# fgnt/padertorch

Measured on AMD Instinct MI355X. Metric: training frames/sec (PIT mask-est, 2-spk 8 kHz), higher is better.
Workload: dtype f32

## Files before the change

include/ptmi.h:

```cpp
#ifndef PTMI_H_
#define PTMI_H_

#include <stdint.h>

#ifdef __cplusplus
extern "C" {
#endif

#define PTMI_OK 0
#define PTMI_E_INVALID (-1)
#define PTMI_E_UNSUPPORTED (-2)

typedef void* ptmi_stream_t;

const char* ptmi_version(void);
const char* ptmi_error_string(int code);

typedef struct ptmi_stft_geom {
    int32_t size;
    int32_t shift;
    int32_t window_length;
    int32_t pad_left;
    int32_t pad_right;
    int32_t pad;
// ... 111 lines not shown
int ptmi_unit_norm_backward(const float* gy, const float* y, const float* inv_norm, float* dx, int64_t N, int32_t E,
                            int32_t F, float eps, ptmi_stream_t stream);

int64_t ptmi_td_stats_elems(int32_t K);
int64_t ptmi_td_workspace_elems(int64_t batch, int32_t K, int64_t T);
int ptmi_td_pair_stats(const float* est, const float* tgt, const int32_t* lengths, int64_t batch, int32_t K,
                       int64_t T, const int64_t* strides, double* workspace, double* stats,
                       ptmi_stream_t stream);
int ptmi_td_lincomb(const float* x, const float* y, const int32_t* lengths, const float* coef_a,
                    const float* coef_b, const float* coef_c, int64_t batch, int32_t K, int64_t T,
                    const int64_t* strides, float* out, ptmi_stream_t stream);

int ptmi_tas_analysis(const float* x, const float* weight, const float* bias, float* out, int64_t B, int64_t T, int32_t N,
                      int32_t L, int32_t stride, int64_t E, int32_t relu, ptmi_stream_t stream);
int ptmi_tas_synthesis(const float* p, const float* mask, const float* gate, const float* weight, const float* bias, float* y,
                       int32_t K, int64_t B, int32_t N, int32_t L, int32_t stride, int64_t E, int64_t T_out,
                       ptmi_stream_t stream);
int ptmi_tas_masked_decode_backward(const float* gy, const float* mask, const float* encoded, const float* weight, float* dmask,
                                    float* dencoded, int32_t K, int64_t B, int64_t T, int32_t N, int32_t L, int32_t stride,
                                    int64_t E, ptmi_stream_t stream);
int64_t ptmi_tas_wgrad_workspace_elems(int64_t B, int32_t N, int32_t L, int32_t stride, int64_t E);
int ptmi_tas_wgrad(const float* g, const float* mask, const float* gate, const float* x, int32_t K, int64_t B, int64_t T,
                   int32_t N, int32_t L, int32_t stride, int64_t E, float* workspace, float* out, ptmi_stream_t stream);

int64_t ptmi_tcn_depthwise_workspace_elems(int64_t B, int64_t T, int32_t H, int32_t K);
int ptmi_tcn_depthwise_forward(const float* u, const float* slope_in, const float* weight, const float* bias, const float* slope_out,
                               float* v, float* stats, double* workspace, int64_t B, int64_t T, int32_t H, int32_t K,
                               int32_t dilation, float eps, ptmi_stream_t stream);
int ptmi_tcn_depthwise_backward(const float* gv, const float* u, const float* slope_in, const float* weight, const float* bias,
                                const float* slope_out, float* gz, float* gu, float* dparams, double* workspace, int64_t B,
                                int64_t T, int32_t H, int32_t K, int32_t dilation, ptmi_stream_t stream);
int64_t ptmi_tcn_norm_workspace_elems(int64_t B, int64_t T, int32_t C);
int ptmi_tcn_norm_stats(const float* x, float* stats, double* workspace, int64_t B, int64_t T, int32_t C, int32_t rows, float eps,
                        ptmi_stream_t stream);
int ptmi_tcn_norm_apply(const float* x, const float* stats, const float* gamma, const float* beta, float* y, int64_t B, int64_t T,
                        int32_t C, int32_t rows, ptmi_stream_t stream);
int ptmi_tcn_norm_backward(const float* gy, const float* x, const float* stats, const float* gamma, float* dx, float* dparams,
                           float* gsum, double* workspace, int64_t B, int64_t T, int32_t C, int32_t rows, ptmi_stream_t stream);

int64_t ptmi_tasnet_entry_norm_workspace_elems(int64_t B, int32_t N, int64_t E);
int ptmi_tasnet_entry_norm_forward(const float* w, const float* gamma, const float* beta, const void* lengths, int32_t lengths_int64,
                                   float* y, float* stats, int64_t B, int32_t N, int64_t E, float eps, ptmi_stream_t stream);
int ptmi_tasnet_entry_norm_backward(const float* gy, const float* w, const float* stats, const float* gamma, const void* lengths,
                                    int32_t lengths_int64, float* dw, float* dparams, double* workspace, int64_t B, int32_t N,
                                    int64_t E, ptmi_stream_t stream);
int64_t ptmi_tasnet_prelu_workspace_elems(int64_t n);
int ptmi_tasnet_prelu_forward(const float* x, const float* slope, float* y, int64_t n, ptmi_stream_t stream);
int ptmi_tasnet_prelu_backward(const float* g, const float* x, const float* slope, float* gx, float* dslope, double* workspace,
                               int64_t n, ptmi_stream_t stream);
int ptmi_tasnet_mask_head_forward(const float* z, float* m, float* additional, int64_t B, int64_t E, int32_t N, int32_t K, int32_t A,
                                  int32_t activation, ptmi_stream_t stream);
int ptmi_tasnet_mask_head_backward(const float* gm, const float* m, const float* g_additional, float* gz, int64_t B, int64_t E,
                                   int32_t N, int32_t K, int32_t A, int32_t activation, ptmi_stream_t stream);
int64_t ptmi_tasnet_center_workspace_elems(int64_t K, int64_t B, int64_t T_in, int64_t T_out);
int ptmi_tasnet_center(const float* in, float* out, double* workspace, int64_t K, int64_t B, int64_t T_in, int64_t T_out,
                       int32_t backward, ptmi_stream_t stream);

int64_t ptmi_dprnn_num_chunks(int64_t L, int32_t K, int32_t P);
int ptmi_dprnn_tables(const void* lengths, int32_t lengths_int64, int32_t B, int32_t S, int32_t K, int32_t P, int32_t* chunks,
                      int32_t* intra, int32_t* inter, ptmi_stream_t stream);
int32_t ptmi_chunk_lstm_max_hidden(void);
int32_t ptmi_chunk_lstm_max_resident_hidden(void);
int32_t ptmi_chunk_lstm_tile(void);
int ptmi_chunk_lstm_forward(float* gates, const float* w_hh, const float* w_hh_reverse, const float* b_hh, const float* b_hh_reverse,
                            float* h, float* c, const int32_t* table, int32_t nseq, int32_t cap, int32_t H, int32_t ndir,
                            ptmi_stream_t stream);
int ptmi_chunk_lstm_backward(float* gates, const float* dh, const float* w_hh, const float* w_hh_reverse, const float* h, const float* c,
                             float* hprev, const int32_t* table, int32_t nseq, int32_t cap, int32_t H, int32_t ndir,
                             ptmi_stream_t stream);
int64_t ptmi_dprnn_colsum_workspace_elems(int64_t rows, int32_t C);
int ptmi_dprnn_colsum(const float* x, int64_t ld, float* out, float* out2, double* workspace, int64_t rows, int32_t C,
                      ptmi_stream_t stream);
int ptmi_dprnn_norm_residual_forward(const float* z, const float* residual, const float* gamma, const float* beta,
                                     const int32_t* chunks, float* y, float* stats, int64_t rows, int32_t N, int32_t S, int32_t K,
                                     float eps, ptmi_stream_t stream);
int ptmi_dprnn_norm_residual_backward(const float* gy, const float* z, const float* stats, const float* gamma, const int32_t* chunks,
                                      float* dz, float* dresidual, float* dparams, double* workspace, int64_t rows, int32_t N,
                                      int32_t S, int32_t K, ptmi_stream_t stream);
int ptmi_dprnn_segment(const float* x, const int64_t* x_strides, float* seg, int64_t B, int64_t L, int32_t N, int32_t S, int32_t K,
                       int32_t P, ptmi_stream_t stream);
int ptmi_dprnn_overlap_add(const float* seg, const int64_t* seg_strides, float* out, int64_t B, int64_t L_out, int32_t N, int32_t S,
                           int32_t K, int32_t P, int32_t front, ptmi_stream_t stream);

int64_t ptmi_td_rect_workspace_elems(int64_t batch, int32_t M, int32_t K, int64_t T);
int ptmi_td_rect_stats(const float* est, const float* tgt, int64_t batch, int32_t M, int32_t K, int64_t T, const int64_t* strides,
                       double* workspace, double* stats, double* gram, ptmi_stream_t stream);
int ptmi_orpit_select(const double* stats, const double* gram, const int32_t* alive_in, int32_t* alive_out, float* loss,
                      int32_t* choice, float* coef_a, float* coef_b, int64_t batch, int32_t K, int64_t n, ptmi_stream_t stream);
int ptmi_td_rect_lincomb(const float* est, const float* tgt, const float* g, const float* coef_a, const float* coef_b, int64_t batch,
                         int32_t M, int32_t K, int64_t T, const int64_t* strides, float* out, ptmi_stream_t stream);
int64_t ptmi_orpit_flag_workspace_elems(int64_t B, int32_t A, int64_t E);
int ptmi_orpit_flag_forward(const float* additional, const float* weight, const float* bias, const float* mask, const float* encoded,
                            float* pre, float* w, float* flag, double* stat, double* workspace, int64_t B, int32_t A, int64_t E,
                            int32_t N, int32_t K, int32_t k, int32_t weighted, ptmi_stream_t stream);
int ptmi_orpit_flag_backward(const float* gflag, const float* gpre, const float* flag, const double* stat, const float* pre, const float* w,
                             const float* additional, const float* weight, const float* mask, const float* encoded, float* dadditional,
                             float* dparams, float* dmask, float* dencoded, double* workspace, int64_t B, int32_t A, int64_t E, int32_t N,
                             int32_t K, int32_t k, int32_t weighted, ptmi_stream_t stream);

int64_t ptmi_bf_psd_workspace_elems(int64_t B, int32_t C, int64_t T, int64_t F, int32_t M);
int ptmi_bf_psd(const float* Y, const float* mask0, const float* mask1, const int32_t* frames, int64_t B, int32_t C, int64_t T, int64_t F,
                int32_t M, int32_t mask_mode, int32_t normalize, double* workspace, double* psd, ptmi_stream_t stream);
int ptmi_bf_souden(const double* psd_target, const double* psd_noise, int64_t B, int64_t F, int32_t C, int32_t ref_channel, float* w_all,
                   double* numden, float* w, int32_t* ref_out, ptmi_stream_t stream);
int ptmi_bf_apply(const float* w, const float* X, const int32_t* frames, int64_t B, int32_t C, int64_t T, int64_t F, float* Z,
                  ptmi_stream_t stream);

int ptmi_absmax(const float* x, int64_t rows, int64_t cols, int64_t ld, uint32_t* out_bits, ptmi_stream_t stream);
int ptmi_absmax_accumulate(const float* x, int64_t rows, int64_t cols, int64_t ld, uint32_t* inout_bits, ptmi_stream_t stream);

int64_t ptmi_planes_elems(int64_t rows, int64_t k);
int ptmi_pack_planes_t(const float* x, int64_t k_rows, int64_t cols, int64_t ld, const uint32_t* amax, uint16_t* out,
                       ptmi_stream_t stream);
int ptmi_pack_planes_n(const float* x, int64_t rows, int64_t k, int64_t ld, const uint32_t* amax, uint16_t* out,
                       ptmi_stream_t stream);
int64_t ptmi_gemm_planes_workspace_elems(int32_t m, int32_t n, int32_t k, int32_t split_k);
int ptmi_gemm_planes(const uint16_t* a, const uint32_t* amax_a, const uint16_t* b, const uint32_t* amax_b, const float* bias, float* c,
                     int64_t ldc, int32_t m, int32_t n, int32_t k, int32_t accumulate, int32_t split_k, int32_t products,
                     float* workspace, ptmi_stream_t stream);
int ptmi_gemm_planes_relu(const uint16_t* a, const uint32_t* amax_a, const uint16_t* b, const uint32_t* amax_b, const float* bias, float* c,
                          int64_t ldc, int32_t m, int32_t n, int32_t k, int32_t split_k, int32_t products, float* workspace,
                          uint32_t* amax_out, int32_t amax_zeroed, ptmi_stream_t stream);
int ptmi_relu_backward_absmax(const float* g, const float* y, float* out, int64_t rows, int64_t cols, int64_t ld_g, int64_t ld_y,
                              int64_t ld_out, uint32_t* amax_out, int32_t amax_zeroed, ptmi_stream_t stream);
int ptmi_pack_planes_t_bf16(const float* x, int64_t k_rows, int64_t cols, int64_t ld, uint16_t* out, ptmi_stream_t stream);
int ptmi_pack_planes_n_bf16(const float* x, int64_t rows, int64_t k, int64_t ld, uint16_t* out, ptmi_stream_t stream);
int ptmi_pack_planes_into(const float* x, int64_t rows_or_k, int64_t cols, int64_t ld, int32_t transposed, int32_t bf16, const uint32_t* amax,
                          uint16_t* out, int64_t kb_total, int64_t kb_offset, int64_t kb_count, ptmi_stream_t stream);
int ptmi_gemm_planes_bf16(const uint16_t* a, const uint16_t* b, const float* bias, float* c, int64_t ldc, int32_t m, int32_t n,
                          int32_t k, int32_t accumulate, int32_t split_k, int32_t products, float* workspace, ptmi_stream_t stream);
int ptmi_gemm_planes_bf16_two(const uint16_t* a, const uint16_t* b, float* c, float* c2, int32_t m_split, int64_t ldc, int32_t m,
                              int32_t n, int32_t k, int32_t accumulate, int32_t split_k, int32_t products, float* workspace,
                              ptmi_stream_t stream);
int ptmi_gemm_planes_bf16_group(const uint16_t* a, int32_t m, int32_t m_split, const uint16_t* const* b, const int32_t* n, int32_t segments,
                                float* const* c, const int64_t* ldc, int32_t k, int32_t accumulate, int32_t split_k, int32_t products,
                                float* workspace, ptmi_stream_t stream);
int64_t ptmi_gemm_planes_group_workspace_elems(int32_t m, int32_t m_split, const int32_t* n, int32_t segments, float* const* c, int32_t k,
                                               int32_t split_k);
int32_t ptmi_gemm_planes_group_plan(int32_t m, int32_t m_split, const int32_t* n, int32_t segments, float* const* c, int32_t k,
                                    int32_t split_k);
int ptmi_pack_planes_t_bf16_list(const float* const* x, const int64_t* cols, const int64_t* ld, uint16_t* const* out, int32_t sources,
                                 int64_t k_rows, ptmi_stream_t stream);
int32_t ptmi_gemm_planes_plan(int32_t m, int32_t n, int32_t k, int32_t split_k);

int ptmi_lstm_bias_grad_add(const float* db, int32_t ndir, int32_t n, float* const* bias_ih_grad, float* const* bias_hh_grad,
                            ptmi_stream_t stream);
int64_t ptmi_grad_norm_workspace_elems(void);
int ptmi_grad_norm(const float* flat, int64_t n, double* workspace, float* norm_out, ptmi_stream_t stream);
int ptmi_adam_flat(float* flat_grad, float* exp_avg, float* exp_avg_sq, const int64_t* segments, int32_t nseg, int64_t n,
                   const float* norm, float max_norm, const float* found_inf, const float* finite, float* applied,
                   const float* step, double lr, double beta1, double beta2, double eps, double weight_decay, const double* hyper,
                   int32_t zero_grad, ptmi_stream_t stream);

#define PTMI_COMM_ID_BYTES 128
typedef struct ptmi_comm ptmi_comm;
int32_t ptmi_comm_rccl_version(void);
int ptmi_comm_unique_id(uint8_t* id_out );
int ptmi_comm_create(ptmi_comm** comm, int32_t world_size, int32_t rank, const uint8_t* id);
int ptmi_allreduce_sum(ptmi_comm* comm, float* buffer, int64_t n, ptmi_stream_t stream);
int ptmi_comm_destroy(ptmi_comm* comm);

#ifdef __cplusplus
}
#endif
#endif
```

padertorch_amd/_lib.py:

```python
import ctypes
import os
import threading
from ctypes import c_char_p, c_double, c_float, c_int, c_int32, c_int64, c_void_p, POINTER
from pathlib import Path

import torch

_PKG = Path(__file__).resolve().parent
LIB_PATH = _PKG / 'libptmi.so'
if os.environ.get('PTMI_LIB'):
    LIB_PATH = Path(os.environ['PTMI_LIB'])


class StftGeom(ctypes.Structure):
    _fields_ = [('size', c_int32), ('shift', c_int32), ('window_length', c_int32),
                ('pad_left', c_int32), ('pad_right', c_int32), ('pad', c_int32)]


class NormGeom(ctypes.Structure):
    _fields_ = [('rank', c_int32), ('size', c_int64 * 5), ('stat_group_stride', c_int64 * 5),
                ('indep_stride', c_int64 * 5), ('batch_dim', c_int32), ('seq_dim', c_int32)]


_P = c_void_p
_G = POINTER(StftGeom)
_I64P = POINTER(c_int64)

SIGNATURES = {
    'ptmi_version': (c_char_p, []),
    'ptmi_error_string': (c_char_p, [c_int]),
    'ptmi_stft_num_frames': (c_int64, [_G, c_int64]),
    'ptmi_istft_num_samples': (c_int64, [_G, c_int64]),
    'ptmi_stft_forward': (c_int, [_P, c_int64, c_int64, c_int64, _P, _P, _P, _G, c_int64, c_int32,
                                  c_float, _P, _P]),
    'ptmi_istft_forward': (c_int, [_P, c_int64, c_int64, _P, _P, _P, _G, c_int32, c_float, c_int64,
                                   c_int64, c_int64, _P, _P]),
    'ptmi_pit_features': (c_int, [_P, _P, c_int64, c_int32, c_int64, c_int64, _P, _P, _P, _G, c_int64,
                                  _P, _P, _P, _P]),
    'ptmi_pit_features_packed': (c_int, [_P, _P, c_int64, c_int32, c_int64, c_int64, _P, _P, _P, _G, c_int64,
                                         _P, _P, _P, _P, _P, _P, _P]),
    'ptmi_pit_workspace_elems': (c_int64, [c_int64, c_int64, c_int32, c_int32]),
    'ptmi_pit_pairwise_sse': (c_int, [_P, _P, _P, _P, c_int64, c_int64, _I64P, c_int32, c_int32, _P,
                                      _P, _P, _P]),
    'ptmi_pit_assign': (c_int, [_P, c_int64, c_int32, c_int32, c_int32, c_int64, _P, _P, _P, _P, _P]),
    'ptmi_pit_backward': (c_int, [_P, _P, _P, _P, _P, _P, c_int64, c_int64, _I64P, c_int32, c_int32,
                                  c_int32, _P, _P, _P]),
    'ptmi_dc_workspace_elems': (c_int64, [c_int64, c_int64, c_int32]),
    'ptmi_dc_loss_forward': (c_int, [_P, _P, c_int64, c_int64, _I64P, c_int32, c_int32, c_int32, _P, _P, _P, _P, _P, _P]),
    'ptmi_dc_loss_backward': (c_int, [_P, _P, _P, _P, c_int64, c_int64, _I64P, c_int32, c_int32, c_int32, _P, _P, _P]),
    'ptmi_stft_logmel': (c_int, [_P, c_int64, c_int64, c_int64, _P, _P, _P, _G, c_int64, _P, _P, _P, _P,
                                 c_int32, c_int32, c_int32, c_int32, c_float, _P, _P]),
    'ptmi_mel_apply': (c_int, [_P, c_int64, c_int32, _P, _P, _P, _P, c_int32, c_int32, c_int32, c_float, _P, _P]),
    'ptmi_norm_workspace_elems': (c_int64, [POINTER(NormGeom), c_int32]),
    'ptmi_norm_reduce': (c_int, [c_int32, _P, _P, _P, _P, _P, _P, POINTER(NormGeom), c_int32, _P, _P, _P]),
    'ptmi_norm_elementwise': (c_int, [c_int32, _P, _P, _P, _P, _P, _P, _P, _P, _P, POINTER(NormGeom), c_int32,
                                      c_int32, _P, _P]),
    'ptmi_td_stats_elems': (c_int64, [c_int32]),
    'ptmi_td_workspace_elems': (c_int64, [c_int64, c_int32, c_int64]),
    'ptmi_td_pair_stats': (c_int, [_P, _P, _P, c_int64, c_int32, c_int64, _I64P, _P, _P, _P]),
    'ptmi_td_lincomb': (c_int, [_P, _P, _P, _P, _P, _P, c_int64, c_int32, c_int64, _I64P, _P, _P]),
    'ptmi_tas_analysis': (c_int, [_P, _P, _P, _P, c_int64, c_int64, c_int32, c_int32, c_int32, c_int64, c_int32, _P]),
    'ptmi_tas_synthesis': (c_int, [_P, _P, _P, _P, _P, _P, c_int32, c_int64, c_int32, c_int32, c_int32, c_int64, c_int64, _P]),
    'ptmi_tas_masked_decode_backward': (c_int, [_P, _P, _P, _P, _P, _P, c_int32, c_int64, c_int64, c_int32, c_int32, c_int32,
                                                c_int64, _P]),
    'ptmi_tas_wgrad_workspace_elems': (c_int64, [c_int64, c_int32, c_int32, c_int32, c_int64]),
    'ptmi_tas_wgrad': (c_int, [_P, _P, _P, _P, c_int32, c_int64, c_int64, c_int32, c_int32, c_int32, c_int64, _P, _P, _P]),
    'ptmi_tcn_depthwise_workspace_elems': (c_int64, [c_int64, c_int64, c_int32, c_int32]),
    'ptmi_tcn_depthwise_forward': (c_int, [_P, _P, _P, _P, _P, _P, _P, _P, c_int64, c_int64, c_int32, c_int32, c_int32, c_float, _P]),
    'ptmi_tcn_depthwise_backward': (c_int, [_P, _P, _P, _P, _P, _P, _P, _P, _P, _P, c_int64, c_int64, c_int32, c_int32, c_int32, _P]),
    'ptmi_tcn_norm_workspace_elems': (c_int64, [c_int64, c_int64, c_int32]),
    'ptmi_tcn_norm_stats': (c_int, [_P, _P, _P, c_int64, c_int64, c_int32, c_int32, c_float, _P]),
    'ptmi_tcn_norm_apply': (c_int, [_P, _P, _P, _P, _P, c_int64, c_int64, c_int32, c_int32, _P]),
    'ptmi_tcn_norm_backward': (c_int, [_P, _P, _P, _P, _P, _P, _P, _P, c_int64, c_int64, c_int32, c_int32, _P]),
    'ptmi_tasnet_entry_norm_workspace_elems': (c_int64, [c_int64, c_int32, c_int64]),
    'ptmi_tasnet_entry_norm_forward': (c_int, [_P, _P, _P, _P, c_int32, _P, _P, c_int64, c_int32, c_int64, c_float, _P]),
    'ptmi_tasnet_entry_norm_backward': (c_int, [_P, _P, _P, _P, _P, c_int32, _P, _P, _P, c_int64, c_int32, c_int64, _P]),
    'ptmi_tasnet_prelu_workspace_elems': (c_int64, [c_int64]),
    'ptmi_tasnet_prelu_forward': (c_int, [_P, _P, _P, c_int64, _P]),
    'ptmi_tasnet_prelu_backward': (c_int, [_P, _P, _P, _P, _P, _P, c_int64, _P]),
    'ptmi_tasnet_mask_head_forward': (c_int, [_P, _P, _P, c_int64, c_int64, c_int32, c_int32, c_int32, c_int32, _P]),
    'ptmi_tasnet_mask_head_backward': (c_int, [_P, _P, _P, _P, c_int64, c_int64, c_int32, c_int32, c_int32, c_int32, _P]),
    'ptmi_tasnet_center_workspace_elems': (c_int64, [c_int64, c_int64, c_int64, c_int64]),
    'ptmi_tasnet_center': (c_int, [_P, _P, _P, c_int64, c_int64, c_int64, c_int64, c_int32, _P]),
    'ptmi_td_rect_workspace_elems': (c_int64, [c_int64, c_int32, c_int32, c_int64]),
    'ptmi_td_rect_stats': (c_int, [_P, _P, c_int64, c_int32, c_int32, c_int64, _I64P, _P, _P, _P, _P]),
    'ptmi_orpit_select': (c_int, [_P, _P, _P, _P, _P, _P, _P, _P, c_int64, c_int32, c_int64, _P]),
    'ptmi_td_rect_lincomb': (c_int, [_P, _P, _P, _P, _P, c_int64, c_int32, c_int32, c_int64, _I64P, _P, _P]),
    'ptmi_orpit_flag_workspace_elems': (c_int64, [c_int64, c_int32, c_int64]),
    'ptmi_orpit_flag_forward': (c_int, [_P, _P, _P, _P, _P, _P, _P, _P, _P, _P, c_int64, c_int32, c_int64, c_int32, c_int32, c_int32,
                                        c_int32, _P]),
    'ptmi_orpit_flag_backward': (c_int, [_P, _P, _P, _P, _P, _P, _P, _P, _P, _P, _P, _P, _P, _P, _P, c_int64, c_int32, c_int64, c_int32,
                                         c_int32, c_int32, c_int32, _P]),
    'ptmi_bf_psd_workspace_elems': (c_int64, [c_int64, c_int32, c_int64, c_int64, c_int32]),
    'ptmi_bf_psd': (c_int, [_P, _P, _P, _P, c_int64, c_int32, c_int64, c_int64, c_int32, c_int32, c_int32, _P, _P, _P]),
    'ptmi_bf_souden': (c_int, [_P, _P, c_int64, c_int64, c_int32, c_int32, _P, _P, _P, _P, _P]),
    'ptmi_bf_apply': (c_int, [_P, _P, _P, c_int64, c_int32, c_int64, c_int64, _P, _P]),
    'ptmi_dprnn_num_chunks': (c_int64, [c_int64, c_int32, c_int32]),
    'ptmi_dprnn_tables': (c_int, [_P, c_int32, c_int32, c_int32, c_int32, c_int32, _P, _P, _P, _P]),
    'ptmi_chunk_lstm_max_hidden': (c_int32, []),
    'ptmi_chunk_lstm_max_resident_hidden': (c_int32, []),
    'ptmi_chunk_lstm_tile': (c_int32, []),
    'ptmi_chunk_lstm_forward': (c_int, [_P, _P, _P, _P, _P, _P, _P, _P, c_int32, c_int32, c_int32, c_int32, _P]),
    'ptmi_chunk_lstm_backward': (c_int, [_P, _P, _P, _P, _P, _P, _P, _P, c_int32, c_int32, c_int32, c_int32, _P]),
    'ptmi_dprnn_colsum_workspace_elems': (c_int64, [c_int64, c_int32]),
    'ptmi_dprnn_colsum': (c_int, [_P, c_int64, _P, _P, _P, c_int64, c_int32, _P]),
    'ptmi_dprnn_norm_residual_forward': (c_int, [_P, _P, _P, _P, _P, _P, _P, c_int64, c_int32, c_int32, c_int32, c_float, _P]),
    'ptmi_dprnn_norm_residual_backward': (c_int, [_P, _P, _P, _P, _P, _P, _P, _P, _P, c_int64, c_int32, c_int32, c_int32, _P]),
    'ptmi_dprnn_segment': (c_int, [_P, _I64P, _P, c_int64, c_int64, c_int32, c_int32, c_int32, c_int32, _P]),
    'ptmi_dprnn_overlap_add': (c_int, [_P, _I64P, _P, c_int64, c_int64, c_int32, c_int32, c_int32, c_int32, c_int32, _P]),
    'ptmi_lstm_forward': (c_int, [_P, _P, _P, _P, _P, _P, _P, c_int32, c_int32, c_int32, c_int32, c_int32, _P]),
    'ptmi_lstm_backward': (c_int, [_P, _P, _P, _P, _P, _P, _P, _P, _P, c_int32, c_int32, c_int32, c_int32, _P]),
    'ptmi_unit_norm_forward': (c_int, [_P, _P, _P, c_int64, c_int32, c_int32, c_float, c_void_p]),
    'ptmi_unit_norm_backward': (c_int, [_P, _P, _P, _P, c_int64, c_int32, c_int32, c_float, c_void_p]),
    'ptmi_lstm_flags_elems': (c_int64, [c_int32, c_int32, c_int32]),
    'ptmi_lstm_scratch_elems': (c_int64, [c_int32, c_int32, c_int32, c_int32, c_int32]),
    'ptmi_lstm_weight_prep': (c_int, [_P, _P, _P, _P, c_int32, c_int32, c_int32, _P, c_int32, _P, _P, c_int32, _P, _P, _P]),
    'ptmi_lstm_set_error_sink': (c_int, [_P]),
    'ptmi_lstm_split_enabled': (c_int, []),
    'ptmi_lstm_handoff_cols': (c_int32, [c_int32, c_int32]),
    'ptmi_lstm_forward_persistent': (c_int, [_P, _P, _P, _P, _P, _P, _P, _P, _P, _P, c_int32, c_int32, c_int64, c_int32, c_int32,
                                             c_int32, c_int32, _P, _P]),
    'ptmi_lstm_forward_fills': (c_int, [c_int32, c_int32, c_int32, c_int32]),
    'ptmi_lstm_backward_planes_ok': (c_int32, [c_int32, c_int32, c_int32, c_int64, c_int32]),
    'ptmi_lstm_backward_persistent': (c_int, [_P, _P, _P, _P, _P, _P, _P, _P, _P, _P, _P, _P, _P, c_int32, c_int32, c_int64, c_int32,
                                              c_int32, c_int32, c_int32, c_int32, _P]),
    'ptmi_absmax': (c_int, [_P, c_int64, c_int64, c_int64, _P, _P]),
    'ptmi_absmax_accumulate': (c_int, [_P, c_int64, c_int64, c_int64, _P, _P]),
    'ptmi_planes_elems': (c_int64, [c_int64, c_int64]),
    'ptmi_pack_planes_t': (c_int, [_P, c_int64, c_int64, c_int64, _P, _P, _P]),
    'ptmi_gemm_planes_workspace_elems': (c_int64, [c_int32, c_int32, c_int32, c_int32]),
    'ptmi_pack_planes_n': (c_int, [_P, c_int64, c_int64, c_int64, _P, _P, _P]),
    'ptmi_gemm_planes': (c_int, [_P, _P, _P, _P, _P, _P, c_int64, c_int32, c_int32, c_int32, c_int32, c_int32, c_int32, _P, _P]),
    'ptmi_gemm_planes_relu': (c_int, [_P, _P, _P, _P, _P, _P, c_int64, c_int32, c_int32, c_int32, c_int32, c_int32, _P, _P, c_int32, _P]),
    'ptmi_relu_backward_absmax': (c_int, [_P, _P, _P, c_int64, c_int64, c_int64, c_int64, c_int64, _P, c_int32, _P]),
    'ptmi_pack_planes_t_bf16': (c_int, [_P, c_int64, c_int64, c_int64, _P, _P]),
    'ptmi_pack_planes_n_bf16': (c_int, [_P, c_int64, c_int64, c_int64, _P, _P]),
    'ptmi_pack_planes_into': (c_int, [_P, c_int64, c_int64, c_int64, c_int32, c_int32, _P, _P, c_int64, c_int64, c_int64, _P]),
    'ptmi_gemm_planes_bf16': (c_int, [_P, _P, _P, _P, c_int64, c_int32, c_int32, c_int32, c_int32, c_int32, c_int32, _P, _P]),
    'ptmi_gemm_planes_bf16_two': (c_int, [_P, _P, _P, _P, c_int32, c_int64, c_int32, c_int32, c_int32, c_int32, c_int32, c_int32, _P, _P]),
    'ptmi_gemm_planes_plan': (c_int32, [c_int32, c_int32, c_int32, c_int32]),
    'ptmi_gemm_planes_bf16_group': (c_int, [_P, c_int32, c_int32, _P, _P, c_int32, _P, _P, c_int32, c_int32, c_int32, c_int32, _P, _P]),
    'ptmi_gemm_planes_group_workspace_elems': (c_int64, [c_int32, c_int32, _P, c_int32, _P, c_int32, c_int32]),
    'ptmi_gemm_planes_group_plan': (c_int32, [c_int32, c_int32, _P, c_int32, _P, c_int32, c_int32]),
    'ptmi_pack_planes_t_bf16_list': (c_int, [_P, _P, _P, _P, c_int32, c_int64, _P]),
    'ptmi_comm_rccl_version': (c_int32, []),
    'ptmi_comm_unique_id': (c_int, [_P]),
    'ptmi_comm_create': (c_int, [_P, c_int32, c_int32, _P]),
    'ptmi_allreduce_sum': (c_int, [_P, _P, c_int64, _P]),
    'ptmi_comm_destroy': (c_int, [_P]),
    'ptmi_lstm_bias_grad_add': (c_int, [_P, c_int32, c_int32, _P, _P, _P]),
    'ptmi_grad_norm_workspace_elems': (c_int64, []),
    'ptmi_grad_norm': (c_int32, [_P, c_int64, _P, _P, _P]),
    'ptmi_adam_flat': (c_int32, [_P, _P, _P, _P, c_int32, c_int64, _P, c_float, _P, _P, _P, _P, c_double, c_double, c_double,
                                 c_double, c_double, _P, c_int32, _P]),
}

_lib = None


def load():
    global _lib
    if _lib is None:
        if not LIB_PATH.exists():
            raise ImportError(
                f'{LIB_PATH} is missing: build the HIP kernels first '
                f'(python -m padertorch_amd.build, or __graft_entry__.build()). '
                f'padertorch_amd has no CPU fallback.')
        lib = ctypes.CDLL(str(LIB_PATH))
        for name, (res, args) in SIGNATURES.items():
            fn = getattr(lib, name)
            fn.restype = res
            fn.argtypes = args
        _lib = lib
    return _lib


_hooks = None


def test_hooks():
    global _hooks
    if _hooks is None:
        path = _PKG / 'libptmi_testhooks.so'
        if not path.exists():
            raise ImportError(f'{path} is missing: python -m padertorch_amd.build')
        lib = ctypes.CDLL(str(path))
        lib.ptmi_test_occupy.restype = c_int
        lib.ptmi_test_occupy.argtypes = [c_int32, c_int32, c_int32, c_int64, _P]
        _hooks = lib
    return _hooks


def select_gemm_tile(tile):
    if tile is None or tile < 0:
        os.environ.pop('PTMI_GEMM_TILE', None)
    else:
        assert 0 <= tile <= 5, tile
        os.environ['PTMI_GEMM_TILE'] = str(int(tile))
    return 0


def check(rc, what=''):
    if rc != 0:
        msg = load().ptmi_error_string(int(rc)).decode()
        raise RuntimeError(f'{what}: {msg} (code {rc})')


def ptr(t):
    return None if t is None else t.data_ptr()


def require_gpu(*tensors):
    for t in tensors:
        if t is not None and not t.is_cuda:
            raise RuntimeError(
                'padertorch_amd ops run on an MI355X (HIP) device only and have no CPU fallback; '
                f'got a tensor on {t.device}. Move the example to the GPU first.')


def stream(device):
    return torch.cuda.current_stream(device).cuda_stream


def device_key(device):
    device = torch.device(device)
    return device.type, device.index if device.index is not None else torch.cuda.current_device()


KERNEL_TIMERS = None


def timed(name, fn, *args):
    if KERNEL_TIMERS is None:
        return fn(*args)
    e0 = torch.cuda.Event(enable_timing=True)
    e1 = torch.cuda.Event(enable_timing=True)
    e0.record()
    rc = fn(*args)
    e1.record()
    KERNEL_TIMERS.append((name, e0, e1))
    return rc


class _Staging:

    def __init__(self, half_bytes=1 << 24):
        self.half = half_bytes
        self.buf = torch.empty(2 * half_bytes, dtype=torch.uint8, pin_memory=True)
        self.np = self.buf.numpy()
        self.which, self.off = 0, 0
        self.events = [[], []]
        self.streams = [{}, {}]
        self.lock = threading.Lock()

    def put(self, t, device):
        n = t.numel() * t.element_size()
        if n > self.half // 4:
            return t.pin_memory().to(device, non_blocking=True)
        with self.lock:
            if self.off + n > self.half:
                for stream in self.streams[self.which].values():
                    ev = torch.cuda.Event()
                    ev.record(stream)
                    self.events[self.which].append(ev)
                self.streams[self.which] = {}
                self.which, self.off = self.which ^ 1, 0
                for ev in self.events[self.which]:
                    ev.synchronize()
                self.events[self.which] = []
            start = self.which * self.half + self.off
            self.off += (n + 63) // 64 * 64
            stage = self.buf[start:start + n].view(t.dtype).view(t.shape)
            self.np[start:start + n] = t.numpy().reshape(-1).view('uint8')
            cur = torch.cuda.current_stream(device)
            self.streams[self.which][cur.cuda_stream] = cur
            return stage.to(device, non_blocking=True)


_STAGING = {}


def host_to_device(values, dtype, device):
    t = torch.as_tensor(values, dtype=dtype)
    device = torch.device(device)
    if device.type != 'cuda' or t.numel() == 0:
        return t.to(device)
    idx = device.index if device.index is not None else torch.cuda.current_device()
    st = _STAGING.get(idx)
    if st is None:
        st = _STAGING[idx] = _Staging()
    return st.put(t.contiguous(), torch.device('cuda', idx))


def strides4(*vals):
    return (c_int64 * 4)(*vals)


def strides6(*vals):
    return (c_int64 * 6)(*vals)


def strides8(*vals):
    return (c_int64 * 8)(*vals)


STRICT = bool(int(os.environ.get('PTMI_STRICT', '0') or 0))
_WARNED = set()

# ... 10 lines not shown
```

padertorch_amd/csrc/gemm_planes.hip:

```cpp
#include <algorithm>

#include "common.h"

namespace ptmi {

typedef _Float16 h8 __attribute__((ext_vector_type(8)));
typedef __bf16 b8 __attribute__((ext_vector_type(8)));
typedef float f4 __attribute__((ext_vector_type(4)));

constexpr int PBM = 128, PBN = 128;
constexpr int FR = 64;

__device__ __forceinline__ float plane_scale(const unsigned* amax_bits) {
    if (!amax_bits) return 1.f;
    const unsigned e = (*amax_bits >> 23) & 0xffu;
    if (e == 0u || e == 0xffu) return 1.f;
    return __uint_as_float((unsigned)(127 + 13 + 127 - (int)e) << 23);
}

struct PlanesArgs {
    const uint4* A;
    const uint4* B;
    float* C;
    float* workspace;
    const unsigned* amax_a;
    const unsigned* amax_b;
    const float* bias;
    int M, N, KB;
    long long ldc;
    int accumulate;
    int kb_per_split;
    int tiles_m, tiles_n;
    float* C2 = nullptr;
    int m_split = 0;
    int relu = 0;
    unsigned* amax_out = nullptr;
};

__device__ __forceinline__ void block_amax(unsigned* out, unsigned m, unsigned* red) {
#pragma unroll
    for (int o = 32; o > 0; o >>= 1) m = max(m, (unsigned)__shfl_xor((int)m, o));
    if ((threadIdx.x & 63) == 0) red[threadIdx.x >> 6] = m;
    __syncthreads();
    if (threadIdx.x == 0) {
        for (unsigned w = 1; w < (blockDim.x >> 6); ++w) m = max(m, red[w]);
        if (m != 0u) atomicMax(out, m >= 0x7f800000u ? 0x7f7fffffu : m);
    }
}

template <bool BF16, bool ONE, bool RELU = false>
__global__ __launch_bounds__(256, 2) void gemm_planes_kernel(const PlanesArgs G) {
#if __HIP_DEVICE_COMPILE__
    constexpr int PIECES = 32;
    __shared__ uint4 lds[2 * PIECES * FR];
    const int tid = threadIdx.x, lane = tid & 63, wave = tid >> 6;
    const int T = G.tiles_m * G.tiles_n;
    const int q = T / 8, r8 = T % 8, xcd = blockIdx.x & 7, idx = blockIdx.x >> 3;
    if (idx >= (xcd < r8 ? q + 1 : q)) return;
    const int tile = (xcd < r8 ? xcd * (q + 1) : r8 * (q + 1) + (xcd - r8) * q) + idx;
    const int tm = tile / G.tiles_n, tn = tile - tm * G.tiles_n;
    const int kb0 = blockIdx.z * G.kb_per_split, kb1 = min(G.KB, kb0 + G.kb_per_split);
    const int wm = wave >> 1, wn = wave & 1;
    const float inv = 1.f / (plane_scale(G.amax_a) * plane_scale(G.amax_b));
    const int rta = (G.M + 15) / 16, rtb = (G.N + 15) / 16;
    const uint4* gsrc[8];
#pragma unroll
    for (int i = 0; i < 8; ++i) {
        const int f = wave * 8 + i;
        const bool isa = f < 16;
        const int rt = (f & 15) >> 1, p = f & 1;
        const long long row_tile = min((long long)(isa ? tm : tn) * 8 + rt, (long long)(isa ? rta : rtb) - 1);
        gsrc[i] = (isa ? G.A : G.B) + ((row_tile * G.KB + kb0) * 2 + p) * FR + lane;
    }
    f4 acc[4][4];
#pragma unroll
    for (int i = 0; i < 4; ++i)
#pragma unroll
        for (int j = 0; j < 4; ++j) acc[i][j] = f4{0.f, 0.f, 0.f, 0.f};
    if (kb0 < kb1) {
#pragma unroll
        for (int i = 0; i < 8; ++i)
            if (!ONE || !(i & 1)) __builtin_amdgcn_global_load_lds(gsrc[i], &lds[(wave * 8 + i) * FR], 16, 0, 0);
    }
    for (int kb = kb0; kb < kb1; ++kb) {
        const int st = (kb - kb0) & 1;
        asm volatile("s_waitcnt vmcnt(0)" ::: "memory");
        __builtin_amdgcn_s_barrier();
        const uint4* sa = &lds[(st * PIECES + wm * 8) * FR + lane];
        const uint4* sb = &lds[(st * PIECES + 16 + wn * 8) * FR + lane];
        const bool more = kb + 1 < kb1;
        h8 bh[4], bl[4];
#pragma unroll
        for (int j = 0; j < 4; ++j) {
            bh[j] = __builtin_bit_cast(h8, sb[(j * 2 + 0) * FR]);
            bl[j] = ONE ? bh[j] : __builtin_bit_cast(h8, sb[(j * 2 + 1) * FR]);
        }
        h8 ah = __builtin_bit_cast(h8, sa[0]), al = ONE ? ah : __builtin_bit_cast(h8, sa[FR]);
#pragma unroll
        for (int i = 0; i < 4; ++i) {
            h8 nh = ah, nl = al;
            if (i + 1 < 4) {
                nh = __builtin_bit_cast(h8, sa[((i + 1) * 2 + 0) * FR]);
                nl = ONE ? nh : __builtin_bit_cast(h8, sa[((i + 1) * 2 + 1) * FR]);
            }
            if (more) {
#pragma unroll
                for (int pc = 2 * i; pc < 2 * i + 2; ++pc)
                    if (!ONE || !(pc & 1))
                        __builtin_amdgcn_global_load_lds(gsrc[pc] + (long long)(kb + 1 - kb0) * 2 * FR,
                                                         &lds[((st ^ 1) * PIECES + wave * 8 + pc) * FR], 16, 0, 0);
            }
#pragma unroll
            for (int p = ONE ? 2 : 0; p < 3; ++p)
#pragma unroll
                for (int j = 0; j < 4; ++j)
                    acc[i][j] = BF16 ? __builtin_amdgcn_mfma_f32_16x16x32_bf16(__builtin_bit_cast(b8, p == 0 ? bl[j] : bh[j]),
                                                                               __builtin_bit_cast(b8, p == 1 ? al : ah), acc[i][j], 0, 0, 0)
                                     : __builtin_amdgcn_mfma_f32_16x16x32_f16(p == 0 ? bl[j] : bh[j], p == 1 ? al : ah, acc[i][j], 0, 0, 0);
            ah = nh;
            al = nl;
        }
    }
    const bool slab = gridDim.z > 1;
    float* const Cz = slab ? G.workspace + (long long)blockIdx.z * G.M * G.N : G.C;
    const long long ldc = slab ? G.N : G.ldc;
    const bool vec = (ldc & 3) == 0 && ((reinterpret_cast<unsigned long long>(Cz) | reinterpret_cast<unsigned long long>(G.C2)) & 15) == 0;
    const bool add = G.accumulate && !slab;
    const int r = lane & 15, g = lane >> 4;
    f4 bv[4];
    {
        const bool bias_on = G.bias != nullptr && !slab;
        const bool bvec = (reinterpret_cast<unsigned long long>(G.bias) & 15) == 0;
#pragma unroll
        for (int j = 0; j < 4; ++j) {
            const int n = tn * PBN + wn * 64 + j * 16 + g * 4;
            bv[j] = f4{0.f, 0.f, 0.f, 0.f};
            if (bias_on && bvec && n + 3 < G.N) {
                bv[j] = *reinterpret_cast<const f4*>(G.bias + n);
            } else if (bias_on) {
#pragma unroll
                for (int e = 0; e < 4; ++e) bv[j][e] = G.bias[min(n + e, G.N - 1)];
            }
        }
    }
    const bool fuse = RELU && !slab;
    unsigned mx = 0u;
#pragma unroll
    for (int i = 0; i < 4; ++i) {
        const int m = tm * PBM + wm * 64 + i * 16 + r;
        if (m >= G.M) continue;
        const bool second = !slab && G.C2 != nullptr && m >= G.m_split;
        float* const rowp = second ? G.C2 + (long long)(m - G.m_split) * ldc : Cz + (long long)m * ldc;
#pragma unroll
        for (int j = 0; j < 4; ++j) {
            const int n = tn * PBN + wn * 64 + j * 16 + g * 4;
            float* o = rowp + n;
            f4 v = acc[i][j] * inv + bv[j];
            if (RELU && fuse) {
#pragma unroll
                for (int e = 0; e < 4; ++e) {
                    v[e] = v[e] < 0.f ? 0.f : v[e];
                    if (n + e < G.N) mx = max(mx, __float_as_uint(v[e]));
                }
            }
// ... 237 lines not shown
            if (GROUP || G.splits > 1) {
                const int sM = GROUP ? bk.rows : G.M, sN = GROUP ? bk.cols : G.N;
                float* const srow = GROUP ? G.slabs + bk.slab + tz * bk.slab_stride + (long long)mrow * sN + n0
                                          : G.slabs + ((long long)tz * G.M + mrow) * G.N + n0;
                const bool svec = (sN & 3) == 0 && (reinterpret_cast<unsigned long long>(G.slabs) & 15) == 0;
                const bool sfull = svec && (tn * WN + wn + 1) * NT * 16 <= sN;
#pragma unroll
                for (int i = 0; i < MT; ++i) {
                    const bool ok = mrow + i * 16 < sM;
#pragma unroll
                    for (int j = 0; j < NT; ++j) {
                        const f4 v = acc[i][j] * inv;
                        acc[i][j] = f4{0.f, 0.f, 0.f, 0.f};
                        float* o = srow + (long long)i * 16 * sN + j * 16;
                        if (sfull) {
                            if (ok) *reinterpret_cast<f4*>(o) = v;
                        } else {
#pragma unroll
                            for (int e = 0; e < 4; ++e)
                                if (ok && n0 + j * 16 + e < sN) o[e] = v[e];
                        }
                    }
                }
                if (!has_next_tile) break;
                idx = nidx;
                tm = ntm;
                tn = ntn;
                tz = ntz;
                if constexpr (GROUP) bk = nbk;
                continue;
            }
            auto rowp = [&](int i) {
                const int m = mrow + i * 16;
                return (G.C2 != nullptr && m >= G.m_split ? G.C2 + (long long)(m - G.m_split) * G.ldc : G.C + (long long)m * G.ldc) + n0;
            };
            if (RELU) {
#pragma unroll
                for (int i = 0; i < MT; ++i) {
                    const bool ok = mrow + i * 16 < G.M;
#pragma unroll
                    for (int j = 0; j < NT; ++j) {
                        f4 v = acc[i][j] * inv + bv[j];
                        acc[i][j] = f4{0.f, 0.f, 0.f, 0.f};
#pragma unroll
                        for (int e = 0; e < 4; ++e) {
                            v[e] = v[e] < 0.f ? 0.f : v[e];
                            if (ok && n0 + j * 16 + e < G.N) relu_max = max(relu_max, __float_as_uint(v[e]));
                        }
                        float* o = rowp(i) + j * 16;
                        if (full) {
                            if (ok) *reinterpret_cast<f4*>(o) = v;
                        } else {
#pragma unroll
                            for (int e = 0; e < 4; ++e)
                                if (ok && n0 + j * 16 + e < G.N) o[e] = v[e];
                        }
                    }
                }
            } else if (full && !G.accumulate) {
#pragma unroll
                for (int i = 0; i < MT; ++i) {
#pragma unroll
                    for (int j = 0; j < NT; ++j) {
                        const f4 v = acc[i][j] * inv + bv[j];
                        acc[i][j] = f4{0.f, 0.f, 0.f, 0.f};
                        if (mrow + i * 16 < G.M) *reinterpret_cast<f4*>(rowp(i) + j * 16) = v;
                    }
                }
            } else if (full) {
#pragma unroll
                for (int i = 0; i < MT; ++i) {
                    const bool ok = mrow + i * 16 < G.M;
                    f4 old[NT];
#pragma unroll
                    for (int j = 0; j < NT; ++j)
                        old[j] = ok ? *reinterpret_cast<const f4*>(rowp(i) + j * 16) : f4{0.f, 0.f, 0.f, 0.f};
#pragma unroll
                    for (int j = 0; j < NT; ++j) {
                        const f4 v = acc[i][j] * inv + bv[j] + old[j];
                        acc[i][j] = f4{0.f, 0.f, 0.f, 0.f};
                        if (ok) *reinterpret_cast<f4*>(rowp(i) + j * 16) = v;
                    }
                }
            } else {
#pragma unroll
                for (int i = 0; i < MT; ++i) {
                    const bool ok = mrow + i * 16 < G.M;
#pragma unroll
                    for (int j = 0; j < NT; ++j) {
                        const f4 v = acc[i][j] * inv + bv[j];
                        acc[i][j] = f4{0.f, 0.f, 0.f, 0.f};
                        float* o = rowp(i) + j * 16;
#pragma unroll
                        for (int e = 0; e < 4; ++e)
                            if (ok && n0 + j * 16 + e < G.N) o[e] = G.accumulate ? o[e] + v[e] : v[e];
                    }
                }
            }
        }
        if (!has_next_tile) break;
        idx = nidx;
        tm = ntm;
        tn = ntn;
        tz = ntz;
    }
    asm volatile("s_waitcnt vmcnt(0)" ::: "memory");
    if constexpr (RELU) {
        if (G.amax_out && G.splits == 1) {
            __shared__ unsigned red[8];
            block_amax(G.amax_out, relu_max, red);
        }
    }
#endif
}

__global__ __launch_bounds__(256) void absmax_kernel(const float* __restrict__ x, long long rows, long long cols, long long ld,
                                                     unsigned* __restrict__ out) {
    __shared__ unsigned red[4];
    const long long n = rows * cols;
    unsigned m = 0u;
    if (ld == cols && (cols & 3) == 0 && (reinterpret_cast<uintptr_t>(x) & 15) == 0) {
        const long long n4 = n >> 2, stride = (long long)gridDim.x * 256;
        const f4* x4 = reinterpret_cast<const f4*>(x);
        long long i = blockIdx.x * 256ll + threadIdx.x;
        for (; i + 3 * stride < n4; i += 4 * stride) {
            const f4 v0 = x4[i], v1 = x4[i + stride], v2 = x4[i + 2 * stride], v3 = x4[i + 3 * stride];
#pragma unroll
            for (int q = 0; q < 4; ++q)
                m = max(max(m, __float_as_uint(v0[q]) & 0x7fffffffu),
                        max(max(__float_as_uint(v1[q]) & 0x7fffffffu, __float_as_uint(v2[q]) & 0x7fffffffu), __float_as_uint(v3[q]) & 0x7fffffffu));
        }
        for (; i < n4; i += stride) {
            const f4 v = x4[i];
#pragma unroll
            for (int q = 0; q < 4; ++q) m = max(m, __float_as_uint(v[q]) & 0x7fffffffu);
        }
    } else {
        for (long long i = blockIdx.x * 256ll + threadIdx.x; i < n; i += (long long)gridDim.x * 256) {
            const long long r = i / cols, c = i - r * cols;
            m = max(m, __float_as_uint(x[r * ld + c]) & 0x7fffffffu);
        }
    }
#pragma unroll
    for (int o = 32; o > 0; o >>= 1) m = max(m, (unsigned)__shfl_xor((int)m, o));
    if ((threadIdx.x & 63) == 0) red[threadIdx.x >> 6] = m;
    __syncthreads();
    if (threadIdx.x == 0) {
        m = max(max(red[0], red[1]), max(red[2], red[3]));
        if (m >= 0x7f800000u) m = 0x7f7fffffu;
        atomicMax(out, m);
    }
}

template <bool BF16>
__device__ __forceinline__ void split_chunk(const float (&v)[8], uint4* hi_out, uint4* lo_out) {
    if (BF16) {
        b8 hi, lo;
#pragma unroll
        for (int e = 0; e < 8; ++e) {
            hi[e] = (__bf16)v[e];
            lo[e] = (__bf16)(v[e] - (float)hi[e]);
        }
        *hi_out = __builtin_bit_cast(uint4, hi);
        *lo_out = __builtin_bit_cast(uint4, lo);
    } else {
        h8 hi, lo;
#pragma unroll
        for (int e = 0; e < 8; ++e) {
            hi[e] = (_Float16)v[e];
            lo[e] = (_Float16)(v[e] - (float)hi[e]);
        }
        *hi_out = __builtin_bit_cast(uint4, hi);
        *lo_out = __builtin_bit_cast(uint4, lo);
    }
}

__global__ __launch_bounds__(256) void planes_reduce_kernel(const float* __restrict__ ws, int splits, float* __restrict__ C, long long ldc,
                                                            const float* __restrict__ bias, int M, int N, int accumulate,
                                                            float* __restrict__ C2 = nullptr, int m_split = 0, int relu = 0,
                                                            unsigned* __restrict__ amax_out = nullptr) {
    const long long total = (long long)M * N;
    unsigned mx = 0u;
    for (long long i = blockIdx.x * 256ll + threadIdx.x; i < total; i += (long long)gridDim.x * 256) {
        const int r = (int)(i / N), c = (int)(i - (long long)r * N);
        float sum = 0.f;
        for (int z = 0; z < splits; ++z) sum += ws[(long long)z * total + i];
        if (bias) sum += bias[c];
        if (relu) {
            sum = sum < 0.f ? 0.f : sum;
            mx = max(mx, __float_as_uint(sum));
        }
        float* o = (C2 != nullptr && r >= m_split) ? C2 + (long long)(r - m_split) * ldc + c : C + (long long)r * ldc + c;
        *o = accumulate ? *o + sum : sum;
    }
    if (relu && amax_out) {
        __shared__ unsigned red[4];
        block_amax(amax_out, mx, red);
    }
}

struct ReduceGroupArgs {
    const float* ws;
    int splits, nblocks, accumulate;
    long long start[GROUP_BLOCKS + 1];
    long long slab_off[GROUP_BLOCKS], slab_stride[GROUP_BLOCKS];
    float* C[GROUP_BLOCKS];
    long long ldc[GROUP_BLOCKS];
    int cols[GROUP_BLOCKS];
    int vec[GROUP_BLOCKS];
};

__global__ __launch_bounds__(256) void planes_reduce_kernel(const ReduceGroupArgs R) {
    const long long total = R.start[R.nblocks];
    for (long long i = blockIdx.x * 256ll + threadIdx.x; i < total; i += (long long)gridDim.x * 256) {
        int b = 0;
#pragma unroll
        for (int q = 1; q < GROUP_BLOCKS; ++q) b += (q < R.nblocks && i >= R.start[q]) ? 1 : 0;
        const int N = R.cols[b];
        const long long stride = R.slab_stride[b];
        if (R.vec[b]) {
            const long long j = (i - R.start[b]) * 4;
            const int r = (int)(j / N), c = (int)(j - (long long)r * N);
            const float* w = R.ws + R.slab_off[b] + j;
            f4 sum = {0.f, 0.f, 0.f, 0.f};
            for (int z = 0; z < R.splits; ++z) sum += *reinterpret_cast<const f4*>(w + (long long)z * stride);
            f4* o = reinterpret_cast<f4*>(R.C[b] + (long long)r * R.ldc[b] + c);
            *o = R.accumulate ? *o + sum : sum;
        } else {
            const long long j = i - R.start[b];
            const int r = (int)(j / N), c = (int)(j - (long long)r * N);
            const float* w = R.ws + R.slab_off[b] + j;
            float sum = 0.f;
            for (int z = 0; z < R.splits; ++z) sum += w[(long long)z * stride];
            float* o = R.C[b] + (long long)r * R.ldc[b] + c;
            *o = R.accumulate ? *o + sum : sum;
        }
    }
}

__global__ __launch_bounds__(256) void relu_backward_absmax_kernel(const float* __restrict__ g, const float* __restrict__ y, float* __restrict__ out,
                                                                   long long rows, long long cols, long long ld_g, long long ld_y, long long ld_o,
                                                                   unsigned* __restrict__ amax_out) {
    unsigned mx = 0u;
    const long long n = rows * cols;
    if (ld_g == cols && ld_y == cols && ld_o == cols && (cols & 3) == 0 &&
        ((reinterpret_cast<uintptr_t>(g) | reinterpret_cast<uintptr_t>(y) | reinterpret_cast<uintptr_t>(out)) & 15) == 0) {
        const long long n4 = n >> 2, stride = (long long)gridDim.x * 256;
        const f4* g4 = reinterpret_cast<const f4*>(g);
        const f4* y4 = reinterpret_cast<const f4*>(y);
        f4* o4 = reinterpret_cast<f4*>(out);
        long long i = blockIdx.x * 256ll + threadIdx.x;
        for (; i + stride < n4; i += 2 * stride) {
            const f4 ga = g4[i], ya = y4[i], gb = g4[i + stride], yb = y4[i + stride];
            f4 va, vb;
#pragma unroll
            for (int q = 0; q < 4; ++q) {
                va[q] = ya[q] <= 0.f ? 0.f : ga[q];
                vb[q] = yb[q] <= 0.f ? 0.f : gb[q];
                mx = max(mx, max(__float_as_uint(va[q]) & 0x7fffffffu, __float_as_uint(vb[q]) & 0x7fffffffu));
            }
            o4[i] = va;
            o4[i + stride] = vb;
        }
        for (; i < n4; i += stride) {
            const f4 ga = g4[i], ya = y4[i];
            f4 va;
#pragma unroll
            for (int q = 0; q < 4; ++q) {
                va[q] = ya[q] <= 0.f ? 0.f : ga[q];
                mx = max(mx, __float_as_uint(va[q]) & 0x7fffffffu);
            }
            o4[i] = va;
        }
    } else {
        for (long long i = blockIdx.x * 256ll + threadIdx.x; i < n; i += (long long)gridDim.x * 256) {
            const long long r = i / cols, c = i - r * cols;
            const float v = y[r * ld_y + c] <= 0.f ? 0.f : g[r * ld_g + c];
            out[r * ld_o + c] = v;
            mx = max(mx, __float_as_uint(v) & 0x7fffffffu);
        }
    }
    __shared__ unsigned red[4];
    block_amax(amax_out, mx, red);
}

template <bool BF16>
__global__ __launch_bounds__(256) void pack_planes_t_kernel(const float* __restrict__ x, long long krows, long long cols, long long ld,
                                                            const unsigned* __restrict__ amax, uint4* __restrict__ out, long long KBS,
                                                            long long KBO) {
    __shared__ float tile[32][65];
    const int tid = threadIdx.x;
    const long long kb = blockIdx.x, c0 = (long long)blockIdx.y * 64;
    const float s = plane_scale(amax);
    {
        const int cx = tid & 63, ky = tid >> 6;
#pragma unroll
        for (int p = 0; p < 8; ++p) {
            const long long k = kb * 32 + ky + p * 4, c = c0 + cx;
            tile[ky + p * 4][cx] = (k < krows && c < cols) ? x[k * ld + c] * s : 0.f;
        }
    }
    __syncthreads();
    const int rl = tid >> 6, g = (tid >> 4) & 3, r = tid & 15;
    const long long rt = blockIdx.y * 4 + rl;
    if (rt * 16 >= ((cols + 15) / 16) * 16) return;
    float v[8];
#pragma unroll
    for (int e = 0; e < 8; ++e) v[e] = tile[g * 8 + e][rl * 16 + r];
    uint4* o = out + ((rt * KBS + KBO + kb) * 2) * FR + g * 16 + r;
    split_chunk<BF16>(v, o, o + FR);
}

template <bool BF16>
__device__ __forceinline__ void pack_planes_t4_block(const float* __restrict__ x, long long krows, long long cols, long long ld, float s,
                                                     uint4* __restrict__ out, long long KBS, long long KBO, long long kb, long long cblock,
                                                     bool aligned) {
    constexpr int P = 68;
    __shared__ float tile[32 * P];
    const int tid = threadIdx.x;
    const long long c0 = cblock * 64;
    const int lx = tid & 15, ly = tid >> 4;
    f4 regs[2];
#pragma unroll
    for (int p = 0; p < 2; ++p) {
        const long long k = kb * 32 + ly + p * 16, c = c0 + lx * 4;
        f4 z = {0.f, 0.f, 0.f, 0.f};
        if (k < krows) {
            if (aligned && c + 4 <= cols) {
// ... 584 lines not shown
```

padertorch_amd/csrc/optim.hip:

```cpp
#include "common.h"

namespace ptmi {

constexpr int kNormBlocks = 1024;
constexpr int kMaxSegs = 1024;

struct AdamArgs {
    float* grad;
    float* m;
    float* v;
    const long long* segs;
    int nseg;
    long long n;
    const float* norm;
    float max_norm;
    const float* found_inf;
    const float* finite;
    float* applied;
    const float* step;
    double lr, beta1, beta2;
    double eps, weight_decay;
    const double* hyper;
    int zero_grad;
};

__global__ __launch_bounds__(256) void sumsq_partials_kernel(const float* __restrict__ x, long long n, double* __restrict__ partials) {
    const long long n4 = n >> 2;
    const float4* x4 = reinterpret_cast<const float4*>(x);
    float acc[4] = {0.f, 0.f, 0.f, 0.f};
    const long long per = (n4 + gridDim.x - 1) / gridDim.x;
    const long long lo = per * blockIdx.x, hi = min(n4, lo + per);
    for (long long i = lo + threadIdx.x; i < hi; i += 256) {
        const float4 q = x4[i];
        acc[0] = fmaf(q.x, q.x, acc[0]);
        acc[1] = fmaf(q.y, q.y, acc[1]);
        acc[2] = fmaf(q.z, q.z, acc[2]);
        acc[3] = fmaf(q.w, q.w, acc[3]);
    }
    double s = (double)acc[0] + (double)acc[1] + ((double)acc[2] + (double)acc[3]);
    if (blockIdx.x == gridDim.x - 1 && threadIdx.x < (n & 3)) {
        const float t = x[(n4 << 2) + threadIdx.x];
        s += (double)t * (double)t;
    }
    __shared__ double red[256];
    red[threadIdx.x] = s;
    __syncthreads();
#pragma unroll
    for (int w = 128; w > 0; w >>= 1) {
        if ((int)threadIdx.x < w) red[threadIdx.x] += red[threadIdx.x + w];
        __syncthreads();
    }
    if (threadIdx.x == 0) partials[blockIdx.x] = red[0];
}

__global__ __launch_bounds__(256) void norm_fold_kernel(const double* __restrict__ partials, int nblk, float* __restrict__ norm) {
    __shared__ double red[256];
    double s = 0.0;
    for (int i = threadIdx.x; i < nblk; i += 256) s += partials[i];
    red[threadIdx.x] = s;
    __syncthreads();
#pragma unroll
    for (int w = 128; w > 0; w >>= 1) {
        if ((int)threadIdx.x < w) red[threadIdx.x] += red[threadIdx.x + w];
        __syncthreads();
    }
    if (threadIdx.x == 0) norm[0] = (float)sqrt(red[0]);
}

typedef __attribute__((address_space(1))) float gfloat;
typedef float f32x4v __attribute__((ext_vector_type(4)));
typedef __attribute__((address_space(1))) f32x4v gf32x4;

struct AdamConsts {
    float clip, step_size, bc2_sqrt;
    float beta2f, omb1, omb2, eps, weight_decay;
    bool skip;
};

__device__ __forceinline__ void adam_one(float& p, float& g, float& m, float& v, const AdamConsts& C) {
    float gg = g * C.clip;
    if (C.weight_decay != 0.f) gg = fmaf(C.weight_decay, p, gg);
    m = m + C.omb1 * (gg - m);
    v = C.beta2f * v + C.omb2 * gg * gg;
    const float denom = sqrtf(v) / C.bc2_sqrt + C.eps;
    p -= C.step_size * (m / denom);
}

__global__ __launch_bounds__(256) void adam_flat_kernel(const AdamArgs A) {
    __shared__ long long seg_off[kMaxSegs + 1];
    __shared__ AdamConsts consts;
    for (int i = threadIdx.x; i < A.nseg; i += 256) seg_off[i] = A.segs[3 * i + 1];
    if (threadIdx.x == 0) {
        seg_off[A.nseg] = A.n;
        AdamConsts c;
        c.skip = (A.found_inf != nullptr && A.found_inf[0] != 0.f) || (A.finite != nullptr && !isfinite(A.finite[0])) ||
                 (A.norm != nullptr && !isfinite(A.norm[0]));
        if (blockIdx.x == 0 && A.applied != nullptr) A.applied[0] = c.skip ? 0.f : 1.f;
        double lr = A.lr, beta1 = A.beta1, beta2 = A.beta2, eps = A.eps, wd = A.weight_decay;
        float max_norm = A.max_norm;
        if (A.hyper != nullptr) {
            lr = A.hyper[0]; beta1 = A.hyper[1]; beta2 = A.hyper[2]; eps = A.hyper[3]; wd = A.hyper[4];
            max_norm = (float)A.hyper[5];
        }
        const double t = (double)A.step[0] + 1.0;
        const double bc1 = 1.0 - pow(beta1, t), bc2 = 1.0 - pow(beta2, t);
        c.step_size = (float)(lr / bc1);
        c.bc2_sqrt = (float)sqrt(bc2);
        c.beta2f = (float)beta2;
        c.omb1 = (float)(1.0 - beta1);
        c.omb2 = (float)(1.0 - beta2);
        c.eps = (float)eps;
        c.weight_decay = (float)wd;
        c.clip = 1.f;
        if (A.norm != nullptr) c.clip = fminf(max_norm / (A.norm[0] + 1e-6f), 1.f);
        consts = c;
    }
    __syncthreads();
    const AdamConsts C = consts;
    const long long n4 = (A.n + 3) >> 2;
    for (long long q = (long long)blockIdx.x * 256 + threadIdx.x; q < n4; q += (long long)gridDim.x * 256) {
        const long long i0 = q << 2;
        int lo = 0, hi = A.nseg - 1;
        while (lo < hi) {
            const int mid = (lo + hi + 1) >> 1;
            if (seg_off[mid] <= i0) lo = mid; else hi = mid - 1;
        }
        const bool full = i0 + 4 <= A.n;
        if (full && i0 + 4 <= seg_off[lo + 1]) {
            gfloat* pp = reinterpret_cast<gfloat*>(static_cast<unsigned long long>(A.segs[3 * lo])) + (i0 - seg_off[lo]);
            float4 g = *reinterpret_cast<float4*>(A.grad + i0);
            if (!C.skip) {
                float4 m = *reinterpret_cast<float4*>(A.m + i0), v = *reinterpret_cast<float4*>(A.v + i0);
                const bool al = (reinterpret_cast<unsigned long long>(pp) & 15) == 0;
                float4 p;
                if (al) {
                    const f32x4v q = *reinterpret_cast<gf32x4*>(pp);
                    p = float4{q[0], q[1], q[2], q[3]};
                } else {
                    p = float4{pp[0], pp[1], pp[2], pp[3]};
                }
                adam_one(p.x, g.x, m.x, v.x, C);
                adam_one(p.y, g.y, m.y, v.y, C);
                adam_one(p.z, g.z, m.z, v.z, C);
                adam_one(p.w, g.w, m.w, v.w, C);
                if (al) *reinterpret_cast<gf32x4*>(pp) = f32x4v{p.x, p.y, p.z, p.w};
                else { pp[0] = p.x; pp[1] = p.y; pp[2] = p.z; pp[3] = p.w; }
                *reinterpret_cast<float4*>(A.m + i0) = m;
                *reinterpret_cast<float4*>(A.v + i0) = v;
            }
            if (A.zero_grad) *reinterpret_cast<float4*>(A.grad + i0) = float4{0.f, 0.f, 0.f, 0.f};
        } else {
            int s = lo;
            for (int e = 0; e < 4 && i0 + e < A.n; ++e) {
                const long long i = i0 + e;
                while (i >= seg_off[s + 1]) ++s;
                if (!C.skip) {
                    gfloat* pp = reinterpret_cast<gfloat*>(static_cast<unsigned long long>(A.segs[3 * s])) + (i - seg_off[s]);
                    float p = *pp, g = A.grad[i], m = A.m[i], v = A.v[i];
                    adam_one(p, g, m, v, C);
                    *pp = p;
                    A.m[i] = m;
                    A.v[i] = v;
                }
                if (A.zero_grad) A.grad[i] = 0.f;
            }
        }
    }
}

struct BiasGradArgs {
    const float* db;
    float* out[4];
    int ndir, n;
};

__global__ void bias_grad_add_kernel(const BiasGradArgs A) {
    const int i = blockIdx.x * blockDim.x + threadIdx.x;
    const int d = blockIdx.y;
    if (i >= A.n) return;
    const float g = A.db[(size_t)d * A.n + i];
    A.out[2 * d][i] += g;
    A.out[2 * d + 1][i] += g;
}

}

extern "C" int ptmi_lstm_bias_grad_add(const float* db, int32_t ndir, int32_t n, float* const* bias_ih_grad, float* const* bias_hh_grad,
                                       ptmi_stream_t stream) {
    PTMI_RETURN_IF(!db || !bias_ih_grad || !bias_hh_grad || (ndir != 1 && ndir != 2) || n < 1, PTMI_E_INVALID);
    ptmi::BiasGradArgs A{db, {nullptr, nullptr, nullptr, nullptr}, ndir, n};
    for (int d = 0; d < ndir; ++d) {
        PTMI_RETURN_IF(!bias_ih_grad[d] || !bias_hh_grad[d], PTMI_E_INVALID);
        A.out[2 * d] = bias_ih_grad[d];
        A.out[2 * d + 1] = bias_hh_grad[d];
    }
    hipLaunchKernelGGL(ptmi::bias_grad_add_kernel, dim3((unsigned)((n + 255) / 256), (unsigned)ndir), dim3(256), 0,
                       static_cast<hipStream_t>(stream), A);
    return ptmi::launch_status();
}

namespace ptmi {

}

using namespace ptmi;

extern "C" {

int64_t ptmi_grad_norm_workspace_elems(void) { return kNormBlocks; }

int ptmi_grad_norm(const float* flat, int64_t n, double* workspace, float* norm_out, ptmi_stream_t stream) {
    PTMI_RETURN_IF(flat == nullptr || workspace == nullptr || norm_out == nullptr || n < 0, PTMI_E_INVALID);
    PTMI_RETURN_IF((reinterpret_cast<uintptr_t>(flat) & 15) != 0, PTMI_E_INVALID);
    hipStream_t st = static_cast<hipStream_t>(stream);
    hipLaunchKernelGGL(sumsq_partials_kernel, dim3(kNormBlocks), dim3(256), 0, st, flat, (long long)n, workspace);
    hipLaunchKernelGGL(norm_fold_kernel, dim3(1), dim3(256), 0, st, workspace, kNormBlocks, norm_out);
    return launch_status();
}

int ptmi_adam_flat(float* flat_grad, float* exp_avg, float* exp_avg_sq, const int64_t* segments, int32_t nseg, int64_t n,
                   const float* norm, float max_norm, const float* found_inf, const float* finite, float* applied, const float* step,
                   double lr, double beta1, double beta2, double eps, double weight_decay, const double* hyper, int32_t zero_grad,
                   ptmi_stream_t stream) {
    PTMI_RETURN_IF(flat_grad == nullptr || exp_avg == nullptr || exp_avg_sq == nullptr || segments == nullptr || step == nullptr,
                   PTMI_E_INVALID);
    PTMI_RETURN_IF(nseg < 1 || n < 1, PTMI_E_INVALID);
    PTMI_RETURN_IF(nseg > kMaxSegs, PTMI_E_UNSUPPORTED);
    PTMI_RETURN_IF(((reinterpret_cast<uintptr_t>(flat_grad) | reinterpret_cast<uintptr_t>(exp_avg) |
                     reinterpret_cast<uintptr_t>(exp_avg_sq)) & 15) != 0, PTMI_E_INVALID);
    PTMI_RETURN_IF((reinterpret_cast<uintptr_t>(hyper) & 7) != 0, PTMI_E_INVALID);
    AdamArgs A{flat_grad, exp_avg, exp_avg_sq, reinterpret_cast<const long long*>(segments), nseg, (long long)n, norm, max_norm,
               found_inf, finite, applied, step, lr, beta1, beta2, eps, weight_decay, hyper, zero_grad};
    const long long n4 = (n + 3) >> 2;
    const long long blocks = (n4 + 255) / 256;
    const int grid = (int)(blocks < 8192 ? blocks : 8192);
    hipLaunchKernelGGL(adam_flat_kernel, dim3(grid), dim3(256), 0, static_cast<hipStream_t>(stream), A);
    return launch_status();
}

}
```

padertorch_amd/ops/gemm.py:

```python
import ctypes
import os
import threading
import weakref

import torch

from .. import _lib
from . import library

__all__ = ['mm', 'absmax', 'weight_absmax', 'UNIT_RANGE', 'PRODUCTS', 'ENABLED', 'usable']

ENABLED = True

PRODUCTS = 3

UNIT_RANGE = 'unit'

_WEIGHT_AMAX = {}


def _refs(params):
    return tuple(weakref.ref(p) for p in params)


def _same(refs, params):
    return refs is not None and len(refs) == len(params) and all(r() is p for r, p in zip(refs, params))


_UPDATED = {}


def note_update(params):
    params = [p for p in params if p.is_cuda]
    if not params:
        return
    ev = torch.cuda.Event()
    ev.record(torch.cuda.current_stream(params[0].device))
    _UPDATED[params[0].device] = (ev, {id(p): (weakref.ref(p), p._version) for p in params})


def update_event(params):
    hit = _UPDATED.get(params[0].device) if params else None
    if hit is None:
        return None
    for p in params:
        e = hit[1].get(id(p))
        if e is None or e[0]() is not p or e[1] != p._version:
            return None
    return hit[0]


def invalidate():
    _WEIGHT_AMAX.clear()
    _WEIGHT_PLANES.clear()
    _UPDATED.clear()
    _KNOWN.clear()
    from . import lstm_forms as _forms
    _forms.clear()


def reset_step():
    known = dict(_KNOWN)
    invalidate()
    _KNOWN.update(known)
    _WAITED.clear()


class _Words(threading.local):
    def __init__(self):
        self.blocks = {}


_WORDS = _Words()


def zero_word(device):
    from . import capture as _capture
    if _capture.ACTIVE:
        return _capture.zero_word(device)
    key = (device.type, device.index, torch.cuda.current_stream(device).cuda_stream)
    ent = _WORDS.blocks.get(key)
    if ent is None or ent[1] >= 64:
        ent = _WORDS.blocks[key] = [torch.zeros(64, dtype=torch.int32, device=device), 0]
    ent[1] += 1
    return ent[0][ent[1] - 1:ent[1]]


def absmax(x):
    assert x.dim() == 2 and x.dtype == torch.float32
    _lib.require_gpu(x)
    if x.stride(1) == 1 or x.shape[1] == 1:
        rows, cols, ld = x.shape[0], x.shape[1], x.stride(0)
    else:
        assert x.stride(0) == 1, x.stride()
        rows, cols, ld = x.shape[1], x.shape[0], x.stride(1)
    return torch.ops.ptmi.absmax(x, rows, cols, max(ld, cols))


_KNOWN = {}
_WAITED = {}


class _Prefetching(threading.local):
    event = None

    def __getitem__(self, _):
        return self.event

    def __setitem__(self, _, value):
        self.event = value


_PREFETCHING = _Prefetching()


def _cached(cache, key, p, make, limit, form=None):
    hit = cache.get(key)
    if hit is not None and hit[0] == p._version and hit[1] == p.data_ptr() and _same(hit[3], (p,)):
        if hit[4] is not None and hit[4] is not _PREFETCHING[0]:
            cur = torch.cuda.current_stream(p.device)
            if _WAITED.get(cur.cuda_stream) is not hit[4]:
                cur.wait_event(hit[4])
                _WAITED[cur.cuda_stream] = hit[4]
        return hit[2]
    if len(cache) > limit:
        cache.clear()
    with torch.no_grad():
        v = make()
    cache[key] = (p._version, p.data_ptr(), v, _refs((p,)), _PREFETCHING[0])
    if form is not None:
        known = _KNOWN.get(id(p))
        if known is None or known[0]() is not p:
            if len(_KNOWN) > 256:
                _KNOWN.clear()
            known = _KNOWN[id(p)] = (weakref.ref(p), set())
        known[1].add(form)
    return v


def prefetch_known(device, everything=False):
    todo = []
    updated = _UPDATED.get(device)
    covered = updated[1] if updated is not None else {}
    for pid, (ref, forms) in list(_KNOWN.items()):
        q = ref()
        if q is None:
            del _KNOWN[pid]
        elif q.device == device and q.dim() == 2:
            e = covered.get(id(q))
            if everything or (e is not None and e[0]() is q and e[1] == q._version):
                todo.append((q, sorted(forms, key=str)))
    if not todo or _PREFETCHING[0] is not None:
        return
    ev = _PREFETCHING[0] = torch.cuda.Event()
    try:
        for q, forms in todo:
            for form in forms:
                if form == 'n':
                    weight_planes(q)
                elif form == 't':
                    weight_planes_t(q)
                else:
                    weight_planes_h(q, *form[1:])
    finally:
        _PREFETCHING[0] = None
        ev.record(torch.cuda.current_stream(device))


def weight_absmax(p):
    return _cached(_WEIGHT_AMAX, id(p), p, lambda: absmax(p.detach() if p.dim() == 2 else p.detach().reshape(-1, p.shape[-1])), 256)


def weights_absmax(params):
    params = tuple(params)
    if len(params) == 1:
        return weight_absmax(params[0])
    key = tuple(id(p) for p in params)
    sig = tuple((p._version, p.data_ptr()) for p in params)
    hit = _WEIGHT_AMAX.get(key)
    if hit is not None and hit[0] == sig and _same(hit[3], params):
        return hit[2]
    v = weight_absmax(params[0])
    for p in params[1:]:
        v = torch.maximum(v, weight_absmax(p))
    _WEIGHT_AMAX[key] = (sig, None, v, _refs(params))
    return v


def seed_weights_absmax(params, word):
    params = tuple(params)
    if len(_WEIGHT_AMAX) > 256:
        _WEIGHT_AMAX.clear()
    if len(params) == 1:
        p = params[0]
        _WEIGHT_AMAX[id(p)] = (p._version, p.data_ptr(), word, _refs((p,)), None)
    else:
        _WEIGHT_AMAX[tuple(id(p) for p in params)] = (tuple((p._version, p.data_ptr()) for p in params), None, word, _refs(params))


PLANES = True


def planes_enabled():
    return ENABLED and PLANES


def pack_t(x, amax=None):
    assert x.dim() == 2 and (x.stride(1) == 1 or x.shape[1] == 1) and x.dtype == torch.float32, (x.shape, x.stride(), x.dtype)
    ax = None if amax is UNIT_RANGE else (absmax(x) if amax is None else amax)
    return torch.ops.ptmi.pack_planes_t(x, ax), ax


def pack_n(x, amax=None):
    assert x.dim() == 2 and (x.stride(1) == 1 or x.shape[1] == 1) and x.dtype == torch.float32, (x.shape, x.stride(), x.dtype)
    ax = None if amax is UNIT_RANGE else (absmax(x) if amax is None else amax)
    return torch.ops.ptmi.pack_planes_n(x, ax), ax
# ... 140 lines not shown
```

padertorch_amd/ops/library.py:

```python
import ctypes
from typing import List, Optional, Tuple

import torch
from torch import Tensor

from .. import _lib

_LIBRARY = torch.library.Library('ptmi', 'DEF')


def _register(schema):
    name = schema.split('(', 1)[0].strip()

    def deco(fn):
        _LIBRARY.define(schema)
        _LIBRARY.impl(name, fn, 'CUDA')
        return getattr(torch.ops.ptmi, name)
    return deco


def _geom(g: List[int]):
    return _lib.StftGeom(*[int(v) for v in g])


# ... 481 lines not shown

@_register('bf_psd(Tensor observation, Tensor? mask0, Tensor? mask1, Tensor? frames, bool normalize) -> Tensor')
def bf_psd(observation, mask0, mask1, frames, normalize):
    lib = _lib.load()
    B, C, T, F = _bf_spectrum(observation)
    masks = [m for m in (mask0, mask1) if m is not None]
    assert mask0 is not None or mask1 is None
    _f32c(*masks)
    mode = 0 if not masks else masks[0].dim() - 2
    assert all(tuple(m.shape) == ((B, C, T, F) if mode == 2 else (B, T, F)) for m in masks), ([m.shape for m in masks], observation.shape)
    M = max(len(masks), 1)
    dev = observation.device
    psd = _doubles(M * B * F * C * C * 2, dev).view(M, B, F, C, C, 2)
    ws = _doubles(lib.ptmi_bf_psd_workspace_elems(B, C, T, F, M), dev)
    _lib.check(_lib.timed('bf_psd', lib.ptmi_bf_psd, observation.data_ptr(), _lib.ptr(mask0), _lib.ptr(mask1), _bf_frames(frames, B),
                          B, C, T, F, M, mode, int(normalize), ws.data_ptr(), psd.data_ptr(), _lib.stream(dev)), 'ptmi_bf_psd')
    return torch.view_as_complex(psd)


@_register('bf_souden(Tensor target_psd, Tensor noise_psd, int ref_channel) -> (Tensor, Tensor, Tensor)')
def bf_souden(target_psd, noise_psd, ref_channel):
    for p in (target_psd, noise_psd):
        assert p.dim() == 4 and p.dtype == torch.complex128 and p.is_contiguous() and p.shape == target_psd.shape, (p.shape, p.dtype)
    B, F, C, _ = target_psd.shape
    assert target_psd.shape[3] == C and ref_channel < C, (target_psd.shape, ref_channel)
    dev = target_psd.device
    w_all = torch.empty((B, F, C, C), dtype=torch.complex64, device=dev)
    w = torch.empty((B, F, C), dtype=torch.complex64, device=dev)
    ref = torch.empty(B, dtype=torch.int32, device=dev)
    numden = _doubles(B * F * C * 2 if ref_channel < 0 else 0, dev)
    _lib.check(_lib.timed('bf_souden', _lib.load().ptmi_bf_souden, target_psd.data_ptr(), noise_psd.data_ptr(), B, F, C,
                          max(int(ref_channel), -1), w_all.data_ptr(), numden.data_ptr() if ref_channel < 0 else None, w.data_ptr(),
                          ref.data_ptr(), _lib.stream(dev)), 'ptmi_bf_souden')
    return w, w_all, ref


@_register('bf_apply(Tensor vector, Tensor mix, Tensor? frames) -> Tensor')
def bf_apply(vector, mix, frames):
    B, C, T, F = _bf_spectrum(mix)
    assert vector.shape == (B, F, C) and vector.dtype == torch.complex64 and vector.is_contiguous(), (vector.shape, vector.dtype)
    out = torch.empty((B, T, F), dtype=torch.complex64, device=mix.device)
    _lib.check(_lib.timed('bf_apply', _lib.load().ptmi_bf_apply, vector.data_ptr(), mix.data_ptr(), _bf_frames(frames, B), B, C, T, F,
                          out.data_ptr(), _lib.stream(mix.device)), 'ptmi_bf_apply')
    return out


_ZERO_WORDS = {}


def _zero_word(device):
    from . import capture as _capture
    if _capture.ACTIVE:
        return _capture.zero_word(device, 256)
    key = (device.index, torch.cuda.current_stream(device).cuda_stream)
    pool = _ZERO_WORDS.get(key)
    if pool is None or pool[1] >= pool[0].numel():
        if len(_ZERO_WORDS) > 16:
            _ZERO_WORDS.clear()
        pool = _ZERO_WORDS[key] = [torch.zeros(256, dtype=torch.int32, device=device), 0]
    pool[1] += 1
    return pool[0][pool[1] - 1:pool[1]]


@_register('absmax(Tensor x, int rows, int cols, int ld) -> Tensor')
def absmax(x, rows, cols, ld):
    out = _zero_word(x.device)
    _lib.check(_lib.load().ptmi_absmax_accumulate(x.data_ptr(), rows, cols, ld, out.data_ptr(), _lib.stream(x.device)), 'ptmi_absmax')
    return out


def _lstm_backward_persistent(gates, c, c0, dhy, w_hh_t, dg, dg_t, scratch, dc_carry, bs_dev, offs_dev, T, max_batch, rows, H, ndir,
                              s_begin, s_end, prefilled, step_masks=None, dc_n=None):
    rc = _lib.timed('lstm_backward', _lib.load().ptmi_lstm_backward_persistent, gates.data_ptr(), c.data_ptr(), _lib.ptr(c0),
                    dhy.data_ptr(), _lib.ptr(dc_n), w_hh_t.data_ptr(), _lib.ptr(dg), _lib.ptr(dg_t), bs_dev.data_ptr(), offs_dev.data_ptr(),
                    _lib.ptr(step_masks), scratch.data_ptr(), _lib.ptr(dc_carry), T, max_batch, rows, H, ndir, s_begin, s_end,
                    int(prefilled), _lib.stream(gates.device))
    if rc == -2:
        return False
    _lib.check(rc, 'ptmi_lstm_backward_persistent')
    return True


@_register('lstm_recurrence_backward_range(Tensor gates, Tensor c, Tensor? c0, Tensor dhy, Tensor w_hh_t, Tensor(a!) dg, '
           'Tensor(b!) scratch, Tensor(c!) dc_carry, Tensor bs_dev, Tensor offs_dev, int T, int max_batch, int rows, int H, '
           'int ndir, int s_begin, int s_end, int prefilled=0, Tensor? dc_n=None) -> bool')
def lstm_recurrence_backward_range(gates, c, c0, dhy, w_hh_t, dg, scratch, dc_carry, bs_dev, offs_dev, T, max_batch, rows, H, ndir,
                                   s_begin, s_end, prefilled=0, dc_n=None):
    assert dc_n is None or (dc_n.shape == (ndir, max_batch, H) and dc_n.is_contiguous()), dc_n.shape
    return _lstm_backward_persistent(gates, c, c0, dhy, w_hh_t, dg, None, scratch, dc_carry, bs_dev, offs_dev, T, max_batch, rows, H, ndir,
                                     s_begin, s_end, prefilled, dc_n=dc_n)


@_register('lstm_recurrence_backward_planes(Tensor gates, Tensor c, Tensor? c0, Tensor dhy, Tensor w_hh_t, Tensor(a!)? dg, '
           'Tensor(b!) dg_t, Tensor(c!) scratch, Tensor(d!)? dc_carry, Tensor bs_dev, Tensor offs_dev, int T, int max_batch, int rows, '
           'int H, int ndir, int s_begin, int s_end, int prefilled=0, Tensor? step_masks=None) -> bool')
def lstm_recurrence_backward_planes(gates, c, c0, dhy, w_hh_t, dg, dg_t, scratch, dc_carry, bs_dev, offs_dev, T, max_batch, rows, H, ndir,
                                    s_begin, s_end, prefilled=0, step_masks=None):
    need = ndir * int(_lib.load().ptmi_planes_elems(4 * H, (s_end - s_begin) * max_batch))
    assert dg_t.dtype == torch.bfloat16 and dg_t.numel() >= need, (dg_t.dtype, dg_t.numel(), need)
    return _lstm_backward_persistent(gates, c, c0, dhy, w_hh_t, dg, dg_t, scratch, dc_carry, bs_dev, offs_dev, T, max_batch, rows, H, ndir,
                                     s_begin, s_end, prefilled, step_masks=step_masks)


@_register('lstm_bias_grad_add_(Tensor db, Tensor(a!)[] bias_ih_grad, Tensor(b!)[] bias_hh_grad) -> ()')
def lstm_bias_grad_add_(db, bias_ih_grad, bias_hh_grad):
    ndir = len(bias_ih_grad)
    n = bias_ih_grad[0].numel()
    assert db.numel() == ndir * n and db.dtype == torch.float32 and db.is_contiguous()
    assert all(t.is_contiguous() and t.numel() == n and t.dtype == torch.float32 for t in list(bias_ih_grad) + list(bias_hh_grad))
    ih = (ctypes.c_void_p * ndir)(*[t.data_ptr() for t in bias_ih_grad])
    hh = (ctypes.c_void_p * ndir)(*[t.data_ptr() for t in bias_hh_grad])
    _lib.check(_lib.load().ptmi_lstm_bias_grad_add(db.data_ptr(), ndir, n, ih, hh, _lib.stream(db.device)), 'ptmi_lstm_bias_grad_add')


@_register('lstm_weight_prep(Tensor[] w_ih, Tensor[] w_hh, Tensor[] b_ih, Tensor[] b_hh, int KP) -> '
           '(Tensor, Tensor, Tensor, Tensor, Tensor)')
def lstm_weight_prep(w_ih, w_hh, b_ih, b_hh, KP):
    ndir, (G, I), H = len(w_ih), w_ih[0].shape, w_hh[0].shape[1]
    dev = w_ih[0].device
    Ipad = (I + 3) // 4 * 4
    f32 = dict(dtype=torch.float32, device=dev)
    w_ih_cat, bias = torch.empty((ndir * G, Ipad), **f32), torch.empty(ndir * G, **f32)
    w_pad, w_t = torch.empty((ndir, G, KP), **f32), torch.empty((ndir, H, G), **f32)
    amax = torch.empty(2, dtype=torch.int32, device=dev)
    ptrs = [(ctypes.c_void_p * ndir)(*[t.data_ptr() for t in ts]) for ts in (w_ih, w_hh, b_ih, b_hh)]
    _lib.check(_lib.timed('lstm_weight_prep', _lib.load().ptmi_lstm_weight_prep, *ptrs, ndir, H, I, w_ih_cat.data_ptr(), Ipad,
                          bias.data_ptr(), w_pad.data_ptr(), KP, w_t.data_ptr(), amax.data_ptr(), _lib.stream(dev)),
               'ptmi_lstm_weight_prep')
    return w_ih_cat, bias, w_pad, w_t, amax


@_register('grad_norm(Tensor flat) -> Tensor')
def grad_norm(flat):
    lib = _lib.load()
    ws = torch.empty(int(lib.ptmi_grad_norm_workspace_elems()), dtype=torch.float64, device=flat.device)
    out = torch.empty((), dtype=torch.float32, device=flat.device)
    _lib.check(_lib.timed('grad_norm', lib.ptmi_grad_norm, flat.data_ptr(), flat.numel(), ws.data_ptr(), out.data_ptr(),
                          _lib.stream(flat.device)), 'ptmi_grad_norm')
    return out


@_register('adam_flat_(Tensor(a!) flat_grad, Tensor(b!) exp_avg, Tensor(c!) exp_avg_sq, Tensor segments, Tensor(d!)[] params, '
           'Tensor? norm, float max_norm, Tensor? found_inf, Tensor? finite, Tensor step, float lr, float beta1, float beta2, '
           'float eps, float weight_decay, bool zero_grad, Tensor? hyper=None) -> Tensor')
def adam_flat_(flat_grad, exp_avg, exp_avg_sq, segments, params, norm, max_norm, found_inf, finite, step, lr, beta1, beta2, eps,
               weight_decay, zero_grad, hyper=None):
    if hyper is not None:
        assert hyper.dtype == torch.float64 and hyper.numel() >= 6 and hyper.device == flat_grad.device and hyper.is_contiguous(), hyper
    applied = torch.empty((), dtype=torch.float32, device=flat_grad.device)
    _lib.check(_lib.timed('adam_flat', _lib.load().ptmi_adam_flat, flat_grad.data_ptr(), exp_avg.data_ptr(),
                          exp_avg_sq.data_ptr(), segments.data_ptr(), segments.shape[0], flat_grad.numel(), _lib.ptr(norm),
                          max_norm, _lib.ptr(found_inf), _lib.ptr(finite), applied.data_ptr(), step.data_ptr(), lr, beta1, beta2,
                          eps, weight_decay, _lib.ptr(hyper), int(zero_grad), _lib.stream(flat_grad.device)), 'ptmi_adam_flat')
    return applied


@_register('pack_planes_t(Tensor x, Tensor? amax) -> Tensor')
def pack_planes_t(x, amax):
    lib = _lib.load()
    k, c = x.shape
    out = torch.empty(int(lib.ptmi_planes_elems(c, k)), dtype=torch.float16, device=x.device)
    _lib.check(_lib.timed(f'pack_planes_t:{k}x{c}', lib.ptmi_pack_planes_t, x.data_ptr(), k, c, _ld(x), _lib.ptr(amax), out.data_ptr(),
                          _lib.stream(x.device)), 'ptmi_pack_planes_t')
    return out


@_register('pack_planes_n(Tensor x, Tensor? amax) -> Tensor')
def pack_planes_n(x, amax):
    lib = _lib.load()
    r, k = x.shape
    out = torch.empty(int(lib.ptmi_planes_elems(r, k)), dtype=torch.float16, device=x.device)
    _lib.check(_lib.timed(f'pack_planes_n:{r}x{k}', lib.ptmi_pack_planes_n, x.data_ptr(), r, k, _ld(x), _lib.ptr(amax), out.data_ptr(),
                          _lib.stream(x.device)), 'ptmi_pack_planes_n')
    return out


@_register('gemm_planes_(Tensor(a!) out, Tensor a, Tensor? amax_a, Tensor b, Tensor? amax_b, Tensor? bias, int M, int N, int K, '
           'bool accumulate, int split_k) -> ()')
def gemm_planes_(out, a, amax_a, b, amax_b, bias, M, N, K, accumulate, split_k):
    _gemm_planes_call('ptmi_gemm_planes', 'gemm_planes', out, M, N, K, split_k,
                      (a.data_ptr(), _lib.ptr(amax_a), b.data_ptr(), _lib.ptr(amax_b), _lib.ptr(bias), out.data_ptr(), max(out.stride(0), N),
                       M, N, K, int(accumulate)))


@_register('gemm_planes_relu_(Tensor(a!) out, Tensor a, Tensor? amax_a, Tensor b, Tensor? amax_b, Tensor? bias, int M, int N, int K, '
           'int split_k, Tensor(b!) amax_out) -> ()')
def gemm_planes_relu_(out, a, amax_a, b, amax_b, bias, M, N, K, split_k, amax_out):
    _gemm_planes_call('ptmi_gemm_planes_relu', 'gemm_planes', out, M, N, K, split_k,
                      (a.data_ptr(), _lib.ptr(amax_a), b.data_ptr(), _lib.ptr(amax_b), _lib.ptr(bias), out.data_ptr(), max(out.stride(0), N),
                       M, N, K), (amax_out.data_ptr(), 1))


@_register('relu_backward_absmax(Tensor g, Tensor y, Tensor(a!) amax_out) -> Tensor')
def relu_backward_absmax(g, y, amax_out):
    lib = _lib.load()
    assert g.dim() == 2 and g.shape == y.shape and g.stride(1) == 1 and y.stride(1) == 1
    out = torch.empty((g.shape[0], g.shape[1]), dtype=torch.float32, device=g.device)
    _lib.check(_lib.timed(f'relu_backward_absmax:{g.shape[0]}x{g.shape[1]}', lib.ptmi_relu_backward_absmax, g.data_ptr(), y.data_ptr(),
                          out.data_ptr(), g.shape[0], g.shape[1], _ld(g), _ld(y), _ld(out), amax_out.data_ptr(), 1, _lib.stream(g.device)),
               'ptmi_relu_backward_absmax')
    return out


def _ld(x):
    return x.stride(0) if x.shape[0] > 1 else max(x.stride(0), x.shape[1])


def _products():
    from . import gemm
    return 1 if gemm.PRODUCTS == 1 else 3


def _gemm_planes_call(entry, timer, out, M, N, K, split_k, head, tail=()):
    lib = _lib.load()
    nws = int(lib.ptmi_gemm_planes_workspace_elems(M, N, K, split_k))
    ws = torch.empty(nws, dtype=torch.float32, device=out.device) if nws else None
    _lib.check(_lib.timed(f'{timer}:{M}x{N}x{K}:{split_k}', getattr(lib, entry), *head, split_k, _products(), _lib.ptr(ws), *tail,
                          _lib.stream(out.device)), entry)


@_register('pack_planes_bf16(Tensor x, bool transposed) -> Tensor')
def pack_planes_bf16(x, transposed):
    lib = _lib.load()
    a, b = x.shape
    rows, k = (b, a) if transposed else (a, b)
    out = torch.empty(int(lib.ptmi_planes_elems(rows, k)), dtype=torch.bfloat16, device=x.device)
    fn = lib.ptmi_pack_planes_t_bf16 if transposed else lib.ptmi_pack_planes_n_bf16
    _lib.check(_lib.timed(f'pack_planes_bf16:{a}x{b}', fn, x.data_ptr(), a, b, _ld(x), out.data_ptr(), _lib.stream(x.device)),
               'ptmi_pack_planes_bf16')
    return out


@_register('pack_planes_into_(Tensor(a!) out, Tensor x, Tensor? amax, bool transposed, int kb_total, int kb_offset, int kb_count) -> ()')
def pack_planes_into_(out, x, amax, transposed, kb_total, kb_offset, kb_count):
    lib = _lib.load()
    a, b = x.shape
    rows = b if transposed else a
    assert out.dtype in (torch.float16, torch.bfloat16) and out.numel() >= (rows + 15) // 16 * kb_total * 1024, (out.dtype, out.numel())
    _lib.check(_lib.timed(f'pack_planes_into:{a}x{b}', lib.ptmi_pack_planes_into, x.data_ptr(), a, b, _ld(x), int(transposed),
                          int(out.dtype == torch.bfloat16), _lib.ptr(amax), out.data_ptr(), kb_total, kb_offset, kb_count,
                          _lib.stream(x.device)), 'ptmi_pack_planes_into')


@_register('gemm_planes_bf16_(Tensor(a!) out, Tensor a, int a_offset, Tensor b, Tensor? bias, int M, int N, int K, bool accumulate, '
           'int split_k) -> ()')
def gemm_planes_bf16_(out, a, a_offset, b, bias, M, N, K, accumulate, split_k):
    _gemm_planes_call('ptmi_gemm_planes_bf16', 'gemm_planes_bf16', out, M, N, K, split_k,
                      (a.data_ptr() + a_offset, b.data_ptr(), _lib.ptr(bias), out.data_ptr(), max(out.stride(0), N), M, N, K, int(accumulate)))


@_register('gemm_planes_bf16_two_(Tensor(a!) out, Tensor(b!) out2, Tensor a, int a_offset, Tensor b, int M, int N, int K, bool accumulate, '
           'int split_k) -> ()')
def gemm_planes_bf16_two_(out, out2, a, a_offset, b, M, N, K, accumulate, split_k):
    assert out.shape[0] + out2.shape[0] == M and out.shape[1] == out2.shape[1] == N and out.stride(0) == out2.stride(0), (out.shape, out2.shape)
    _gemm_planes_call('ptmi_gemm_planes_bf16_two', 'gemm_planes_bf16', out, M, N, K, split_k,
                      (a.data_ptr() + a_offset, b.data_ptr(), out.data_ptr(), out2.data_ptr(), out.shape[0], max(out.stride(0), N), M, N, K,
                       int(accumulate)))


@_register('pack_planes_bf16_list(Tensor[] xs) -> Tensor[]')
def pack_planes_bf16_list(xs):
    lib = _lib.load()
    n, k = len(xs), xs[0].shape[0]
    assert 1 <= n <= 3 and all(x.dim() == 2 and x.shape[0] == k and x.dtype == torch.float32 and (x.stride(1) == 1 or x.shape[1] == 1)
                               for x in xs), [tuple(x.shape) for x in xs]
    outs = [torch.empty(int(lib.ptmi_planes_elems(x.shape[1], k)), dtype=torch.bfloat16, device=x.device) for x in xs]
    src = (ctypes.c_void_p * n)(*[x.data_ptr() for x in xs])
    dst = (ctypes.c_void_p * n)(*[o.data_ptr() for o in outs])
    cols = (ctypes.c_int64 * n)(*[x.shape[1] for x in xs])
    ld = (ctypes.c_int64 * n)(*[_ld(x) for x in xs])
    _lib.check(_lib.timed(f'pack_planes_bf16_list:{k}x{sum(x.shape[1] for x in xs)}', lib.ptmi_pack_planes_t_bf16_list, src, cols, ld, dst, n,
                          k, _lib.stream(xs[0].device)), 'ptmi_pack_planes_t_bf16_list')
    return outs


@_register('gemm_planes_bf16_group_(Tensor(a!)[] outs, int[] blocks, Tensor a, int a_offset, int M, int m_split, Tensor[] bs, int[] ns, '
           'int K, bool accumulate, int split_k) -> bool')
def gemm_planes_bf16_group_(outs, blocks, a, a_offset, M, m_split, bs, ns, K, accumulate, split_k):
    lib = _lib.load()
    S = len(bs)
    assert len(outs) == len(blocks) and len(ns) == S and len(set(blocks)) == len(blocks), (len(outs), blocks, ns)
    c = (ctypes.c_void_p * (2 * S))()
    ldc = (ctypes.c_int64 * (2 * S))()
    for o, blk in zip(outs, blocks):
        p, s = divmod(int(blk), S)
        assert p in (0, 1) and o.dtype == torch.float32 and o.shape == ((M - m_split) if p else m_split, ns[s]) and o.stride(1) == 1, \
            (blk, o.shape, o.stride())
        c[blk] = o.data_ptr()
        ldc[blk] = max(o.stride(0), ns[s])
    n = (ctypes.c_int32 * S)(*[int(v) for v in ns])
    b = (ctypes.c_void_p * S)(*[t.data_ptr() for t in bs])
    if int(lib.ptmi_gemm_planes_group_plan(M, m_split, n, S, c, K, split_k)) // 100 == 5:
        return False
    ws = torch.empty(int(lib.ptmi_gemm_planes_group_workspace_elems(M, m_split, n, S, c, K, split_k)), dtype=torch.float32, device=a.device)
    shape = f'{M}/{m_split}x{"+".join(str(int(v)) for v in ns)}x{K}'
    rc = _lib.timed(f'gemm_group_bf16:{shape}:{split_k}', lib.ptmi_gemm_planes_bf16_group, a.data_ptr() + a_offset, M, m_split, b, n, S, c,
                    ldc, K, int(accumulate), split_k, _products(), ws.data_ptr(), _lib.stream(a.device))
    if rc == -2:
        return False
    _lib.check(rc, 'ptmi_gemm_planes_bf16_group')
    return True


@_register('unit_norm_forward(Tensor x, float eps) -> (Tensor, Tensor)')
def unit_norm_forward(x, eps):
    N, E, F = x.shape
# ... 204 lines not shown
```

padertorch_amd/ops/lstm_forms.py:

```python
import torch

from .. import _lib
from . import gemm as _gemm

_STACKED = {}
_PREP_STREAMS = {}
_EARLY_FORK = {}


def clear():
    _STACKED.clear()


def reset_step():
    _EARLY_FORK.clear()


def kpad_of(H):
    return (H + 15) // 16 * 16


def _prep_stream(device, first_layer=False):
    key = _lib.device_key(device) + (bool(first_layer),)
    if key not in _PREP_STREAMS:
        _PREP_STREAMS[key] = torch.cuda.Stream(device=device)
    return _PREP_STREAMS[key]


def begin_captured_step(device):
    from . import capture as _capture
    assert _capture.ACTIVE
    device = torch.device(device)
    pre, pre0 = _prep_stream(device), _prep_stream(device, True)
    pre.wait_stream(torch.cuda.current_stream(device))
    pre0.wait_stream(torch.cuda.current_stream(device))
    _EARLY_FORK[_lib.device_key(device)] = (pre, pre0)


def end_captured_step(device):
    device = torch.device(device)
    for side in _EARLY_FORK.pop(_lib.device_key(device), ()):
        torch.cuda.current_stream(device).wait_stream(side)


def _stacked_stale(params):
    flat = tuple(p for ps in params for p in ps)
    hit = _STACKED.get(tuple(id(p) for p in flat))
    return hit is None or hit[0] != tuple((p._version, p.data_ptr()) for p in flat) or not _gemm._same(hit[2], flat)


class _LazyPlanes:

    def __init__(self, w, amax):
        self.w, self.amax, self.value = w, amax, None

    def get(self):
        if self.value is None:
            with torch.no_grad():
                self.value = _gemm.pack_n(self.w, self.amax)
        return self.value


class LayerForms:

    def __init__(self, w_ih, bias, w_hh, w_pad, w_t, w_ih_kpad, w_ih_planes=None, w_ih_planes_h=None, w_ih_planes_dx=None):
        self.w_ih, self.bias, self.w_hh, self.w_pad, self.w_t, self.w_ih_kpad = w_ih, bias, w_hh, w_pad, w_t, w_ih_kpad
        self.w_ih_planes, self.w_ih_planes_h, self.w_ih_planes_dx = w_ih_planes, w_ih_planes_h, w_ih_planes_dx
        self.ready = None

    def input_planes(self):
        v = self.w_ih_planes
        return v.get() if isinstance(v, _LazyPlanes) else v


def _forms_kernel(params, KP, dx_from_handoff, stream):
    p0 = params[0][0]
    main = torch.cuda.current_stream(p0.device)
    with torch.cuda.stream(stream if stream is not None else main):
        w_ih_k, bias, w_pad, w_t, amax = torch.ops.ptmi.lstm_weight_prep(
            [ps[0].detach() for ps in params], [ps[1].detach() for ps in params], [ps[2].detach() for ps in params],
            [ps[3].detach() for ps in params], KP)
        I, H = p0.shape[1], params[0][1].shape[1]
        planes = planes_h = None
        ndir_ = len(params)
        cols_ = int(_lib.load().ptmi_lstm_handoff_cols(H, 0)) if _gemm.planes_enabled() else 0
        if cols_ and I == ndir_ * H:
            planes_h = ((_gemm.pack_n_direction_blocks(w_ih_k[:, :I], ndir_, H, cols_, amax[0:1]), amax[0:1]), cols_)
            if cols_ == H:
                planes = planes_h[0]
        if _gemm.planes_enabled() and planes is None:
            planes = _gemm.pack_n(w_ih_k[:, :I], amax[0:1]) if planes_h is None else _LazyPlanes(w_ih_k[:, :I], amax[0:1])
        planes_dx = None
        cols_b = int(_lib.load().ptmi_lstm_handoff_cols(H, 1)) if (planes is not None and dx_from_handoff) else 0
        if cols_b and I == ndir_ * H:
            planes_dx = (_gemm.stacked_planes_t_bf16(w_ih_k[:, :I], ndir_, cols_b), cols_b)
    forms = LayerForms(w_ih_k[:, :I], bias, w_pad[:, :, :H], w_pad, w_t, w_ih_k if w_ih_k.shape[1] != I else None,
                       planes, planes_h, planes_dx)
    if stream is not None:
        forms.ready = torch.cuda.Event()
        forms.ready.record(stream)
    _gemm.seed_weights_absmax([ps[0] for ps in params], amax[0:1])
    _gemm.seed_weights_absmax([ps[1] for ps in params], amax[1:2])
    return forms


def _forms_torch(params, KP):
    w_ih = torch.cat([ps[0] for ps in params], 0)
    bias = torch.cat([ps[2] + ps[3] for ps in params], 0)
    w_hh = torch.stack([ps[1] for ps in params], 0)
    H = w_hh.shape[2]
    kpad = -w_ih.shape[1] % 4
    return LayerForms(
        w_ih=w_ih, bias=bias, w_hh=w_hh,
        w_ih_kpad=torch.nn.functional.pad(w_ih, (0, kpad)) if kpad else None,
        w_pad=torch.nn.functional.pad(w_hh, (0, KP - H)).contiguous() if KP != H else w_hh.contiguous(),
        w_t=w_hh.transpose(1, 2).contiguous())


def stacked_weights(params, KP, dx_from_handoff, stream=None):
    key = tuple(id(p) for ps in params for p in ps)
    sig = tuple((p._version, p.data_ptr()) for ps in params for p in ps)
    flat_ps = tuple(p for ps in params for p in ps)
    hit = _STACKED.get(key)
    if hit is not None and hit[0] == sig and _gemm._same(hit[2], flat_ps):
        return hit[1]
    if len(_STACKED) > 64:
        _STACKED.clear()
    with torch.no_grad():
        if params[0][0].is_cuda and all(p.dtype == torch.float32 and p.is_contiguous() for ps in params for p in ps):
            forms = _forms_kernel(params, KP, dx_from_handoff, stream)
        else:
            forms = _forms_torch(params, KP)
    _STACKED[key] = (sig, forms, _gemm._refs(flat_ps))
    return forms


def fork_preparation(all_params, data, H, defer_wgrad, dx_from_handoff):
    flat_params = [p for ps_ in all_params for ps in ps_ for p in ps]
    if not (data.is_cuda and any(_stacked_stale(ps_) for ps_ in all_params)
            and all(p.is_cuda and p.dtype == torch.float32 for p in flat_params)
            and (not (torch.is_grad_enabled() and any(p.requires_grad for p in flat_params))
                 or (defer_wgrad and all(p.requires_grad and p.is_leaf and p.grad is not None for p in flat_params)))):
        return None, None
    pre = _prep_stream(data.device)
    updated = _gemm.update_event(flat_params)
    from . import capture as _capture
    early = _EARLY_FORK.get(_lib.device_key(data.device)) if _capture.ACTIVE else None
    pre0 = early[1] if early else None
    early = bool(early)
    if early:
        pass
    elif updated is not None:
        pre.wait_event(updated)
    else:
        pre.wait_stream(torch.cuda.current_stream(data.device))
    for layer, ps_ in enumerate(all_params):
        if _stacked_stale(ps_) and (layer > 0 or pre0 is not None):
            stacked_weights(ps_, kpad_of(H), dx_from_handoff, stream=pre if layer > 0 else pre0)
    if updated is not None or early:
        with torch.cuda.stream(pre):
            _gemm.prefetch_known(data.device, everything=early)
    return pre, pre0


def join_preparation(device, forked, pre0):
    from . import capture as _capture
    if _capture.ACTIVE and forked is not None:
        torch.cuda.current_stream(device).wait_stream(forked)
        if pre0 is not None:
            torch.cuda.current_stream(device).wait_stream(pre0)
```

padertorch_amd/train/graphed.py:

```python
import numpy as np
import torch

from ..ops import capture as _capture

__all__ = ['GraphedStep', 'signature']


def signature(examples):
    import numpy as np
    from ..ops.sequence.pack_module import PaddedList
    parts = []

    def walk(x):
        if torch.is_tensor(x):
            parts.append(('T', tuple(x.shape), str(x.dtype), str(x.device), tuple(x.stride())))
        elif isinstance(x, PaddedList):
            if not x.intact():
                raise TypeError('edited PaddedList')
            parts.append(('PL', tuple(x.padded.shape), str(x.padded.dtype), str(x.padded.device), tuple(x.lengths), bool(x.batch_first)))
        elif isinstance(x, dict):
            parts.append(('D', tuple(x.keys())))
            for v in x.values():
                walk(v)
        elif isinstance(x, (list, tuple)):
# ... 82 lines not shown
        self.captured_exchange = bool(trainer._dp_active()) and not self.split
        if self.split:
            assert trainer.dp_protocol == 'flat+words' and trainer._buckets is None, \
                "a captured data-parallel step speaks the 'flat+words' protocol (Trainer.dp_protocol; Trainer.train sets it with graph_steps)"
        if self.captured_exchange:
            assert trainer.dp_protocol is None, "graph_exchange = 'captured' keeps the eager loop's collectives (layer buckets, update gate)"
        self.times = None
        self._eager(warmup)
        self._capture()

    @staticmethod
    def _clone(example):
        from ..ops.sequence.pack_module import PaddedList

        def walk(x):
            if torch.is_tensor(x):
                return x.clone()
            if isinstance(x, PaddedList) and x.intact():
                return PaddedList(x.padded.clone(), x.lengths, x.batch_first, x.lengths_dev)
            if hasattr(x, 'static_tensors') and hasattr(x, 'clone'):
                return x.clone()
            if isinstance(x, dict):
                return type(x)((k, walk(v)) for k, v in x.items())
            if isinstance(x, (list, tuple)):
                return type(x)(walk(v) for v in x)
            return x
        return walk(example)

    @staticmethod
    def _tensors(example):
        from ..ops.sequence.pack_module import PaddedList
        out = []

        def walk(x):
            if torch.is_tensor(x):
                out.append(x)
            elif isinstance(x, PaddedList) and x.intact():
                out.append(x.padded)
            elif hasattr(x, 'static_tensors'):
                out.extend(x.static_tensors())
            elif isinstance(x, dict):
                for v in x.values():
                    walk(v)
            elif isinstance(x, (list, tuple)):
                for v in x:
                    walk(v)
        walk(example)
        return out

    @staticmethod
    def _strip_records(example):
        from ..ops.sequence.pack_module import PaddedList

        def walk(x):
            if isinstance(x, PaddedList):
                if getattr(x, 'packed_log1p', None) is not None:
                    x.packed_log1p = None
            elif isinstance(x, dict):
                for v in x.values():
                    walk(v)
            elif isinstance(x, (list, tuple)):
                for v in x:
                    walk(v)
        walk(example)

    def _micro_steps(self):
        tr = self.trainer
        capturing = _capture.ACTIVE
        if capturing:
            from ..ops import lstm as _lstm
            _capture.zero_block(self.device)
            _lstm.begin_captured_step(self.device)
        self._forward_backward()
        if capturing:
            _lstm.end_captured_step(self.device)

    def _forward_backward(self):
        tr = self.trainer
        for i, example in enumerate(self.examples):
            if tr._buckets is not None:
                tr._buckets.active = i + 1 == len(self.examples)
            batch = self.prepare(example) if self.prepare is not None else example
            loss, _, _, review = tr.train_step(tr.model, batch, self.device)
            tr.train_summary.update(review)
            tr.backward(loss)
            del loss, review, batch

    def _one_step(self):
        self._micro_steps()
        return self.trainer.optimizer_step()

    def _eager(self, n):
        tr = self.trainer
        keep = tr.deferred_checks
        tr.deferred_checks = True
        try:
            for _ in range(n):
                self._one_step()
            tr._check_pending(flush=True)
        finally:
            tr.deferred_checks = keep
        torch.cuda.synchronize(self.device)

    def _weight_pattern(self):
        lw = self.trainer.loss_weights
        if lw is None:
            return None
        return tuple((k, 0 if w == 0 else 1 if w == 1 else 2) for k, w in lw.items())

    def _capture(self):
        tr = self.trainer
        assert not tr._dp_active() or self.split or self.captured_exchange
        keep = tr.deferred_checks
        tr._check_pending(flush=True)
        tr.deferred_checks = True
        self._graph = None
        self._stage = tr._graph_stage = _StaticStage(device=self.device)
        opt = tr.optimizer
        device_hyper = hasattr(opt, 'refresh_device_hyper') and getattr(opt, '_native_ok', lambda: False)()
        if device_hyper:
            opt.refresh_device_hyper(self.device)
            opt.hyper_from_device = True
        graph = torch.cuda.CUDAGraph()
        running_summary = tr.train_summary
        tr.train_summary = type(running_summary)()
        opt_step = tr._opt_step
        self._tail = self._words = None
        try:
            from ..ops import lstm as _lstm
            with _capture.capture_mode():
                if not self.split:
                    with torch.cuda.graph(graph, capture_error_mode='thread_local'):
                        self._one_step()
                else:
                    self._words = torch.zeros(2, dtype=torch.float32, device=self.device)
                    with torch.cuda.graph(graph, capture_error_mode='thread_local'):
                        self._micro_steps()
                        _lstm.sync_deferred()
                        self._words.copy_(tr._local_words())
                    self._tail = torch.cuda.CUDAGraph()
                    with torch.cuda.graph(self._tail, pool=graph.pool(), capture_error_mode='thread_local'):
                        tr._exchanged = self._words
                        tr.optimizer_step()
        finally:
            tr._exchanged = None
            tr._graph_stage = None
            tr.deferred_checks = keep
            tr.train_summary = running_summary
            tr._opt_step = opt_step
            if device_hyper:
                opt.hyper_from_device = False
        self._graph = graph
        self._device_hyper = device_hyper
        self._baked = None if device_hyper else self._baked_hyper()
        self._pattern = self._weight_pattern()
        self.captures += 1

    def _baked_hyper(self):
        opt = getattr(self.trainer.optimizer, 'optimizer', None)
        groups = getattr(opt, 'param_groups', None) or []
        return (tuple(tuple(sorted((k, repr(v)) for k, v in g.items() if k != 'params')) for g in groups),
                repr(getattr(self.trainer.optimizer, 'gradient_clipping', None)))

    def _refresh(self):
        tr = self.trainer
        if self._weight_pattern() != self._pattern or (self._baked is not None and self._baked_hyper() != self._baked):
            self._capture()
        if self._device_hyper:
            tr.optimizer.refresh_device_hyper(self.device)
        if tr.loss_weights is not None:
            self._stage.refresh_loss_weights(tr.loss_weights)

    def load(self, examples):
        assert len(examples) == len(self.examples), (len(examples), len(self.examples))
        for example, static in zip(examples, self._inputs):
            new = self._tensors(example)
            assert len(new) == len(static), 'example structure differs from the captured one'
            for src, dst in zip(new, static):
                if src is not dst:
                    assert src.shape == dst.shape and src.dtype == dst.dtype, (src.shape, dst.shape, src.dtype, dst.dtype)
                    dst.copy_(src, non_blocking=True)

    def __call__(self, examples=None, then_load=None):
        tr = self.trainer
        self._refresh()
        if examples is not None and examples is not self.examples:
            self.load(examples)
        if not self.split:
            self._graph.replay()
        else:
            ev = [torch.cuda.Event(enable_timing=True) for _ in range(4)] if self.times is not None else None
            if ev:
                ev[0].record()
            self._graph.replay()
            if ev:
                ev[1].record()
            tr._exchange(self._words)
            if ev:
                ev[2].record()
            self._tail.replay()
            if ev:
                ev[3].record()
        if then_load is not None:
            nxt = then_load() if callable(then_load) else then_load
            if nxt is not None:
                self.load(nxt)
        tr._opt_step += 1
        self._steps += 1
        torch.autograd.graph.increment_version(tr._flat.params)
        torch.cuda.current_stream(self.device).synchronize()
        if self.split and self.times is not None:
            self.times.append(tuple(ev[i].elapsed_time(ev[i + 1]) for i in range(3)))
        jobs = [(what, host, context) for what, host, context, _ in self._stage.jobs]
        self._inspect(jobs)
        self._record_summary(jobs)
        return self._summary()

    def _record_summary(self, jobs):
        for (what, host, context), (_, static_host, _, _) in zip(jobs, self._stage.jobs):
            scalars = {}
            if what == 'loss':
                base = static_host.data_ptr()
                for key, value in context.get('scalars', {}).items():
                    if torch.is_tensor(value) and value.numel() == 1 and value.is_pinned():
                        i = (value.data_ptr() - base) // value.element_size()
                        if 0 <= i < static_host.numel():
                            scalars[key] = float(host.reshape(-1)[i])
                            continue
                    if not torch.is_tensor(value):
                        scalars[key] = value
                lw = self.trainer.loss_weights
                for key in list(scalars):
                    if lw is not None and key.endswith('_loss_weight') and key[:-len('_loss_weight')] in lw:
                        scalars[key] = lw[key[:-len('_loss_weight')]]
            elif what == 'grad_norm':
                scalars['grad_norm'] = float(host[0][0])
                for key, value in context.get('scalars', {}).items():
                    if not torch.is_tensor(value):
                        scalars[key] = value
                groups = getattr(getattr(self.trainer.optimizer, 'optimizer', None), 'param_groups', None) or []
                for i, group in enumerate(groups):
                    scalars[f'lr/param_group_{i}'] = group['lr']
            self.trainer.train_summary.update({'scalars': scalars})

    def _summary(self):
        out = {'scalars': {}, 'histograms': {}}
        for what, host, _, _ in self._stage.jobs:
            if what == 'grad_norm':
                out['scalars']['grad_norm'] = host[0][0]
                out['histograms']['grad_norm_'] = host[0]
        return out

    def _inspect(self, jobs):
        tr = self.trainer
        from ..ops import lstm as _lstm
        for what, host, context in jobs:
            if what == 'loss':
                value = float(host[-1])
                if not np.isfinite(value):
                    path = tr.log_error_state({'state_dict': tr.state_dict(), 'review': context})
                    raise RuntimeError(f'The loss ({value}) is not finite.\n'
                                       f'See error states (model, example, model_out and review) in {path}.')
            elif what == 'grad_norm':
                norm, timeouts = float(host[0][0]), int(host[1][0])
                if _lstm.errors_since_last_report(self.device, timeouts):
                    _lstm.raise_timeout(self.device)
                tr._check_other_ranks_loss(host)
                if not np.isfinite(norm):
                    path = tr.log_error_state({'state_dict': tr.state_dict(), 'optimizer_summary': context})
                    raise RuntimeError(f'The grad_norm ({norm}) is not finite.\n'
                                       f'See error states (model, example, model_out and review) in {path}.')

    def scalars(self):
        out = {}
        for what, host, context, _ in self._stage.jobs:
            if what == 'loss':
                out['loss'] = float(host[-1])
            elif what == 'grad_norm':
                out['grad_norm'] = float(host[0][0])
        return out
```

padertorch_amd/train/optimizer.py:

```python
import os

import torch
from torch import optim

__all__ = ['Optimizer', 'Adam', 'SGD', 'FlatGrads']


class FlatGrads:

    def __init__(self, parameters):
        self.params = [p for p in parameters if p.requires_grad]
        assert self.params, 'no trainable parameters'
        dev, dt = self.params[0].device, self.params[0].dtype
        assert all(p.device == dev and p.dtype == dt for p in self.params), 'mixed device/dtype'
        self.flat = torch.zeros(sum(p.numel() for p in self.params), device=dev, dtype=dt)
        off = 0
        for p in self.params:
            n = p.numel()
            p.grad = self.flat[off:off + n].view_as(p)
            off += n

    def intact(self):
        return all(p.grad is not None and p.grad.untyped_storage().data_ptr()
                   == self.flat.untyped_storage().data_ptr() for p in self.params)


class Optimizer:
    optimizer_cls = None
    optimizer = None
    parameters = None
    flat_grads = None

    def __init__(self, gradient_clipping, **kwargs):
        self.gradient_clipping = gradient_clipping
        self.optimizer_kwargs = kwargs

    def set_parameters(self, parameters):
        self.parameters = tuple(parameters)
        self.optimizer = self.optimizer_cls(self.parameters, **self.optimizer_kwargs)

    def check_if_set(self):
        assert self.optimizer is not None, \
            'The optimizer is not initialized, call set_parameter before' \
            ' using any of the optimizer functions'

    def use_flat_grads(self):
        self.check_if_set()
        self.flat_grads = FlatGrads(self.parameters)
        return self.flat_grads

    def zero_grad(self):
        self.check_if_set()
        if self.flat_grads is not None and self.flat_grads.intact():
            self.flat_grads.flat.zero_()
            return None
        return self.optimizer.zero_grad(set_to_none=False)

    def step(self):
        self.check_if_set()
        return self.optimizer.step()

    def step_and_zero_grad(self):
        self.step()
        self.zero_grad()

    def clip_grad(self):
        self.check_if_set()
        if self.flat_grads is not None and self.flat_grads.intact():
            flat = self.flat_grads.flat
            total_norm = torch.linalg.vector_norm(flat, 2)
            clip_coef = torch.clamp(self.gradient_clipping / (total_norm + 1e-6), max=1.0)
            flat.mul_(clip_coef)
            return total_norm
        return torch.nn.utils.clip_grad_norm_(self.parameters, self.gradient_clipping)

    def _state_tensors(self):
        self.check_if_set()
        for per_param in self.optimizer.state.values():
            for name, value in per_param.items():
                if torch.is_tensor(value):
                    yield per_param, name, value

    def to(self, device):
        if device is not None:
            for per_param, name, value in list(self._state_tensors()):
                per_param[name] = value.to(device)

    def cpu(self):
        return self.to('cpu')

    def cuda(self, device=None):
        assert device is None or isinstance(device, int), device
        return self.to(torch.device('cuda', device) if isinstance(device, int) else torch.device('cuda'))

    def state_dict(self):
        self.check_if_set()
        return self.optimizer.state_dict()

    def load_state_dict(self, state_dict):
        self.check_if_set()
        return self.optimizer.load_state_dict(state_dict)


class Adam(Optimizer):
    optimizer_cls = optim.Adam
    native = True

    def __init__(self, gradient_clipping=1e10, lr=1e-3, betas=(0.9, 0.999), eps=1e-8,
                 weight_decay=0, amsgrad=False):
        super().__init__(gradient_clipping, lr=lr, betas=betas, eps=eps,
                         weight_decay=weight_decay, amsgrad=amsgrad)
        self._bound = None
        self._norm = None
        self.skip_if_not_finite = None
        self._hyper = None
        self.hyper_from_device = False

    def set_parameters(self, parameters):
        self.parameters = tuple(parameters)
        self._bound = None
        try:
            self.optimizer = self.optimizer_cls(self.parameters, fused=True, **self.optimizer_kwargs)
        except (RuntimeError, TypeError, ValueError):
            self.optimizer = self.optimizer_cls(self.parameters, **self.optimizer_kwargs)

    def _native_ok(self):
        fg = self.flat_grads
        if not self.native or fg is None or not fg.flat.is_cuda or fg.flat.dtype != torch.float32 or not fg.intact():
            return False
        groups = self.optimizer.param_groups
        if len(groups) != 1:
            return False
        if len(fg.params) > 1024 or not all(p.is_contiguous() for p in fg.params):
            return False
        g = groups[0]
        return not (g.get('amsgrad') or g.get('maximize') or g.get('differentiable') or g.get('capturable'))

    def _bind(self):
        fg, opt = self.flat_grads, self.optimizer
        keys = tuple(p.data_ptr() for p in fg.params)
        b = self._bound
        if b is not None and b[4] == keys and b[0].device == fg.flat.device and all(
                (st := opt.state.get(p)) is not None and st['exp_avg'].data_ptr() == b[0].data_ptr() + 4 * off
                and st['exp_avg_sq'].data_ptr() == b[1].data_ptr() + 4 * off and st['step'].data_ptr() == b[2].data_ptr() + 4 * i
                for i, (p, off) in enumerate(zip(fg.params, b[5]))):
            return b
        dev = fg.flat.device
        m, v = torch.zeros_like(fg.flat), torch.zeros_like(fg.flat)
        steps = torch.zeros(len(fg.params), dtype=torch.float32, device=dev)
        offs, table, off = [], [], 0
        for i, p in enumerate(fg.params):
            n = p.numel()
            st = opt.state.get(p)
            if st:
                m[off:off + n].copy_(st['exp_avg'].reshape(-1))
                v[off:off + n].copy_(st['exp_avg_sq'].reshape(-1))
                steps[i:i + 1].copy_(torch.as_tensor(st['step'], dtype=torch.float32).reshape(1))
            opt.state[p] = {'step': steps[i], 'exp_avg': m[off:off + n].view_as(p), 'exp_avg_sq': v[off:off + n].view_as(p)}
            table.append((p.data_ptr(), off, n))
            offs.append(off)
            off += n
        segs = torch.tensor(table, dtype=torch.int64).to(dev)
        self._bound = (m, v, steps, segs, keys, offs)
        return self._bound

    def live_hyper(self):
        g = self.optimizer.param_groups[0]
        return (float(g['lr']), float(g['betas'][0]), float(g['betas'][1]), float(g['eps']), float(g['weight_decay']),
                float(self.gradient_clipping))

    def refresh_device_hyper(self, device=None):
        live = self.live_hyper()
        if self._hyper is None or (device is not None and self._hyper[1].device != torch.device(device)):
            device = torch.device(device) if device is not None else self.flat_grads.flat.device
            self._hyper = [torch.zeros(8, dtype=torch.float64, pin_memory=True), torch.zeros(8, dtype=torch.float64, device=device), None]
        host, dev, held = self._hyper
        if held != live:
            if held is not None:
                torch.cuda.current_stream(dev.device).synchronize()
            host[:6] = torch.tensor(live, dtype=torch.float64)
            dev.copy_(host, non_blocking=True)
            self._hyper[2] = live
        return dev

    def clip_grad(self):
        if not self._native_ok():
            return super().clip_grad()
        self._norm = torch.ops.ptmi.grad_norm(self.flat_grads.flat)
        return self._norm

    @torch.no_grad()
    def _native_step(self, zero_grad):
        m, v, steps, segs, _, _ = self._bind()
        fg, opt = self.flat_grads, self.optimizer
        g = opt.param_groups[0]
        found = getattr(opt, 'found_inf', None)
        if found is not None and not (torch.is_tensor(found) and found.is_cuda):
            found = None
        finite, self.skip_if_not_finite = self.skip_if_not_finite, None
        if finite is not None:
            finite = finite.detach().reshape(1).float()
        hyper = self._hyper[1] if self.hyper_from_device else None
        applied = torch.ops.ptmi.adam_flat_(
            fg.flat, m, v, segs, list(fg.params), self._norm, float(self.gradient_clipping),
            None if found is None else found.reshape(1).float(), finite, steps, float(g['lr']), float(g['betas'][0]),
            float(g['betas'][1]), float(g['eps']), float(g['weight_decay']), bool(zero_grad), hyper)
        torch.autograd.graph.increment_version(fg.params)
        from ..ops import gemm as _gemm
        _gemm.note_update(fg.params)
        steps.add_(applied)
        self._norm = None

    def step(self):
        self.check_if_set()
        if not self._native_ok():
            return self.optimizer.step()
        return self._native_step(zero_grad=False)

    def step_and_zero_grad(self):
        self.check_if_set()
        if not self._native_ok():
            return super().step_and_zero_grad()
        return self._native_step(zero_grad=True)

    def zero_grad(self):
        self._norm = None
        return super().zero_grad()


class SGD(Optimizer):
    optimizer_cls = optim.SGD

    def __init__(self, gradient_clipping=1e10, lr=1e-3, momentum=0, dampening=0, weight_decay=0,
                 nesterov=False):
        super().__init__(gradient_clipping, lr=lr, momentum=momentum, dampening=dampening,
                         weight_decay=weight_decay, nesterov=nesterov)
```

Before: 1.239 million.

## Fuse LSTM weight-form packing into the Adam optimizer step kernel

Adds a forms-aware Adam kernel. While it updates the LSTM weights it also writes the derived packed weight forms (padded, transposed, bf16 hi/lo planes and absmax words) that the next forward pass needs. This removes the separate per-step forms-packing kernel launches and the extra re-read of the freshly updated parameters. In exchange it brings host-side planning, owner and registration tables, staleness tracking and a refresh path for graph replay, along with added complexity and risk of stale caches.

After: 1.234 million. No clear change (-0.4%).

```diff
diff --git a/include/ptmi.h b/include/ptmi.h
--- a/include/ptmi.h
+++ b/include/ptmi.h
@@ -287,6 +287,18 @@
                    const float* step, double lr, double beta1, double beta2, double eps, double weight_decay, const double* hyper,
                    int32_t zero_grad, ptmi_stream_t stream);
 
+#define PTMI_ADAM_FORMS_LAYER_WORDS 24
+int ptmi_adam_forms_plan(int64_t* layers, int32_t nlayers, const int64_t* segments, int32_t nseg, int64_t n, int64_t* ranges,
+                         int32_t* nranges, int32_t* counts, int64_t* rest_quads);
+int ptmi_adam_forms_owners(const int64_t* layers, int32_t nlayers, const int64_t* segments, int32_t nseg, int64_t n, int32_t* owner,
+                           int64_t* conflicts);
+int ptmi_adam_flat_forms(float* flat_grad, float* exp_avg, float* exp_avg_sq, const int64_t* segments, int32_t nseg, int64_t n,
+                         const float* norm, float max_norm, const float* found_inf, const float* finite, float* applied,
+                         const float* step, double lr, double beta1, double beta2, double eps, double weight_decay, const double* hyper,
+                         int32_t zero_grad, const int64_t* layers, int32_t nlayers, const int64_t* ranges, int32_t nranges,
+                         int32_t tile_jobs, int32_t rest_blocks, int64_t rest_quads, uint32_t* amax_words, int32_t n_amax_words,
+                         int32_t update, ptmi_stream_t stream);
+
 #define PTMI_COMM_ID_BYTES 128
 typedef struct ptmi_comm ptmi_comm;
 int32_t ptmi_comm_rccl_version(void);
diff --git a/padertorch_amd/_lib.py b/padertorch_amd/_lib.py
--- a/padertorch_amd/_lib.py
+++ b/padertorch_amd/_lib.py
@@ -153,7 +153,14 @@
     'ptmi_grad_norm': (c_int32, [_P, c_int64, _P, _P, _P]),
     'ptmi_adam_flat': (c_int32, [_P, _P, _P, _P, c_int32, c_int64, _P, c_float, _P, _P, _P, _P, c_double, c_double, c_double,
                                  c_double, c_double, _P, c_int32, _P]),
+    'ptmi_adam_forms_plan': (c_int, [_P, c_int32, _P, c_int32, c_int64, _P, _P, _P, _P]),
+    'ptmi_adam_forms_owners': (c_int, [_P, c_int32, _P, c_int32, c_int64, _P, _P]),
+    'ptmi_adam_flat_forms': (c_int32, [_P, _P, _P, _P, c_int32, c_int64, _P, c_float, _P, _P, _P, _P, c_double, c_double, c_double,
+                                       c_double, c_double, _P, c_int32, _P, c_int32, _P, c_int32, c_int32, c_int32, c_int64, _P, c_int32,
+                                       c_int32, _P]),
 }
+
+PTMI_ADAM_FORMS_LAYER_WORDS = 24
 
 _lib = None
 
diff --git a/padertorch_amd/csrc/gemm_planes.hip b/padertorch_amd/csrc/gemm_planes.hip
--- a/padertorch_amd/csrc/gemm_planes.hip
+++ b/padertorch_amd/csrc/gemm_planes.hip
@@ -1,15 +1,13 @@
 #include <algorithm>
 
 #include "common.h"
+#include "planes_chunk.h"
 
 namespace ptmi {
 
-typedef _Float16 h8 __attribute__((ext_vector_type(8)));
-typedef __bf16 b8 __attribute__((ext_vector_type(8)));
 typedef float f4 __attribute__((ext_vector_type(4)));
 
 constexpr int PBM = 128, PBN = 128;
-constexpr int FR = 64;
 
 __device__ __forceinline__ float plane_scale(const unsigned* amax_bits) {
     if (!amax_bits) return 1.f;
@@ -553,28 +551,6 @@
     }
 }
 
-template <bool BF16>
-__device__ __forceinline__ void split_chunk(const float (&v)[8], uint4* hi_out, uint4* lo_out) {
-    if (BF16) {
-        b8 hi, lo;
-#pragma unroll
-        for (int e = 0; e < 8; ++e) {
-            hi[e] = (__bf16)v[e];
-            lo[e] = (__bf16)(v[e] - (float)hi[e]);
-        }
-        *hi_out = __builtin_bit_cast(uint4, hi);
-        *lo_out = __builtin_bit_cast(uint4, lo);
-    } else {
-        h8 hi, lo;
-#pragma unroll
-        for (int e = 0; e < 8; ++e) {
-            hi[e] = (_Float16)v[e];
-            lo[e] = (_Float16)(v[e] - (float)hi[e]);
-        }
-        *hi_out = __builtin_bit_cast(uint4, hi);
-        *lo_out = __builtin_bit_cast(uint4, lo);
-    }
-}
 
 __global__ __launch_bounds__(256) void planes_reduce_kernel(const float* __restrict__ ws, int splits, float* __restrict__ C, long long ldc,
                                                             const float* __restrict__ bias, int M, int N, int accumulate,
diff --git a/padertorch_amd/csrc/optim.hip b/padertorch_amd/csrc/optim.hip
--- a/padertorch_amd/csrc/optim.hip
+++ b/padertorch_amd/csrc/optim.hip
@@ -1,4 +1,9 @@
+#include <algorithm>
+#include <utility>
+#include <vector>
+
 #include "common.h"
+#include "planes_chunk.h"
 
 namespace ptmi {
 
@@ -22,6 +27,11 @@
     double eps, weight_decay;
     const double* hyper;
     int zero_grad;
+    const long long* layers;
+    const long long* ranges;
+    int nlayers, nranges, tile_jobs;
+    long long rest_quads;
+    int update;
 };
 
 __global__ __launch_bounds__(256) void sumsq_partials_kernel(const float* __restrict__ x, long long n, double* __restrict__ partials) {
@@ -70,6 +80,8 @@
 typedef __attribute__((address_space(1))) float gfloat;
 typedef float f32x4v __attribute__((ext_vector_type(4)));
 typedef __attribute__((address_space(1))) f32x4v gf32x4;
+typedef __attribute__((address_space(1))) unsigned guint;
+typedef __attribute__((address_space(1))) u32x4 gu32x4;
 
 struct AdamConsts {
     float clip, step_size, bc2_sqrt;
@@ -77,93 +89,358 @@
     bool skip;
 };
 
+template <bool FUSED>
 __device__ __forceinline__ void adam_one(float& p, float& g, float& m, float& v, const AdamConsts& C) {
+#pragma clang fp contract(off)
     float gg = g * C.clip;
     if (C.weight_decay != 0.f) gg = fmaf(C.weight_decay, p, gg);
-    m = m + C.omb1 * (gg - m);
-    v = C.beta2f * v + C.omb2 * gg * gg;
+    const float d = gg - m, t = (C.omb2 * gg) * gg;
+    if (FUSED) {
+        m = fmaf(C.omb1, d, m);
+        v = fmaf(C.beta2f, v, t);
+    } else {
+        m = m + C.omb1 * d;
+        v = C.beta2f * v + t;
+    }
     const float denom = sqrtf(v) / C.bc2_sqrt + C.eps;
-    p -= C.step_size * (m / denom);
-}
-
-__global__ __launch_bounds__(256) void adam_flat_kernel(const AdamArgs A) {
+    p = fmaf(-C.step_size, m / denom, p);
+}
+
+__host__ __device__ inline bool adam_fused_at(long long i, long long seg_lo, long long seg_hi) {
+    const long long q0 = i & ~3ll;
+    return q0 >= seg_lo && q0 + 4 <= seg_hi;
+}
+
+struct FormGeom {
+    int H, I, KP, G;
+    int tiles_g, strips_h;
+    int ncb, ih_kb;
+    int jobs_hh, jobs_ih, jobs_bias;
+};
+
+__host__ __device__ inline FormGeom form_geom(int H, int I, int KP, int kb_count) {
+    FormGeom g;
+    g.H = H; g.I = I; g.KP = KP; g.G = 4 * H;
+    g.tiles_g = (g.G + 31) / 32;
+    g.strips_h = (KP + 127) / 128;
+    g.ncb = (I + 63) / 64;
+    g.ih_kb = kb_count > 0 ? kb_count : g.tiles_g;
+    g.jobs_hh = g.tiles_g * g.strips_h;
+    g.jobs_ih = g.ncb * g.ih_kb;
+    g.jobs_bias = (g.G + 255) / 256;
+    return g;
+}
+
+__host__ __device__ inline bool form_hh_elem(const FormGeom& g, int job, int tid, int s, int q, int& row, int& col) {
+    const int tg = job / g.strips_h, ts = job - tg * g.strips_h;
+    row = tg * 32 + (tid >> 5) + q * 8;
+    col = ts * 128 + s * 32 + (tid & 31);
+    return row < g.G && col < g.H;
+}
+
+__host__ __device__ inline void form_ih_quad(const FormGeom& g, int job, int tid, int p, int& kb, int& cblock, int& row, int& col) {
+    kb = job / g.ncb;
+    cblock = job - kb * g.ncb;
+    row = kb * 32 + (tid >> 4) + p * 16;
+    col = cblock * 64 + (tid & 15) * 4;
+}
+
+__host__ __device__ inline long long form_rest_quad(const long long* ranges, int nranges, long long rq, long long& vlo, long long& vhi) {
+    int r = 0;
+    while (r + 1 < nranges && rq >= ranges[3 * (r + 1) + 2]) ++r;
+    vlo = ranges[3 * r];
+    vhi = ranges[3 * r + 1];
+    return ((vlo >> 2) + (rq - ranges[3 * r + 2])) << 2;
+}
+
+constexpr int kMaxFormLayers = 64;
+constexpr int kMaxRestRanges = 64;
+enum FormWord {
+    FW_P_WIH = 0, FW_P_WHH, FW_P_BIH, FW_P_BHH,
+    FW_OFF_WIH, FW_OFF_WHH, FW_OFF_BIH, FW_OFF_BHH,
+    FW_H, FW_I, FW_KP, FW_IPAD,
+    FW_W_PAD, FW_W_T, FW_BIAS, FW_AMAX,
+    FW_W_IH_CAT, FW_PLANES_DX,
+    FW_KB_TOTAL, FW_KB_OFFSET, FW_KB_COUNT,
+    FW_JOB_START, FW_JOB_END,
+    FW_RESERVED,
+    FW_WORDS
+};
+static_assert(FW_WORDS == PTMI_ADAM_FORMS_LAYER_WORDS, "include/ptmi.h");
+
+__device__ __forceinline__ void publish_max_global(guint* word, float m, unsigned* red) {
+    unsigned u = __float_as_uint(m);
+#pragma unroll
+    for (int o = 32; o > 0; o >>= 1) u = max(u, (unsigned)__shfl_xor((int)u, o));
+    if ((threadIdx.x & 63) == 0) red[threadIdx.x >> 6] = u;
+    __syncthreads();
+    if (threadIdx.x == 0) {
+        u = max(max(red[0], red[1]), max(red[2], red[3]));
+        if (u >= 0x7f800000u) u = 0x7f7fffffu;
+        if (u > __hip_atomic_load(word, __ATOMIC_RELAXED, __HIP_MEMORY_SCOPE_AGENT))
+            __hip_atomic_fetch_max(word, u, __ATOMIC_RELAXED, __HIP_MEMORY_SCOPE_AGENT);
+    }
+}
+
+__device__ __forceinline__ void adam_quad(const AdamArgs& A, const AdamConsts& C, const long long* seg_off, long long i0, long long vlo,
+                                          long long vhi) {
+    int lo = 0, hi = A.nseg - 1;
+    while (lo < hi) {
+        const int mid = (lo + hi + 1) >> 1;
+        if (seg_off[mid] <= i0) lo = mid; else hi = mid - 1;
+    }
+    const bool full = i0 >= vlo && i0 + 4 <= vhi;
+    if (full && i0 + 4 <= seg_off[lo + 1]) {
+        gfloat* pp = reinterpret_cast<gfloat*>(static_cast<unsigned long long>(A.segs[3 * lo])) + (i0 - seg_off[lo]);
+        float4 g = *reinterpret_cast<float4*>(A.grad + i0);
+        if (!C.skip) {
+            float4 m = *reinterpret_cast<float4*>(A.m + i0), v = *reinterpret_cast<float4*>(A.v + i0);
+            const bool al = (reinterpret_cast<unsigned long long>(pp) & 15) == 0;
+            float4 p;
+            if (al) {
+                const f32x4v q = *reinterpret_cast<gf32x4*>(pp);
+                p = float4{q[0], q[1], q[2], q[3]};
+            } else {
+                p = float4{pp[0], pp[1], pp[2], pp[3]};
+            }
+            adam_one<true>(p.x, g.x, m.x, v.x, C);
+            adam_one<true>(p.y, g.y, m.y, v.y, C);
+            adam_one<true>(p.z, g.z, m.z, v.z, C);
+            adam_one<true>(p.w, g.w, m.w, v.w, C);
+            if (al) *reinterpret_cast<gf32x4*>(pp) = f32x4v{p.x, p.y, p.z, p.w};
+            else { pp[0] = p.x; pp[1] = p.y; pp[2] = p.z; pp[3] = p.w; }
+            *reinterpret_cast<float4*>(A.m + i0) = m;
+            *reinterpret_cast<float4*>(A.v + i0) = v;
+        }
+        if (A.zero_grad) *reinterpret_cast<float4*>(A.grad + i0) = float4{0.f, 0.f, 0.f, 0.f};
+    } else {
+        int s = lo;
+        for (int e = 0; e < 4 && i0 + e < vhi; ++e) {
+            const long long i = i0 + e;
+            if (i < vlo) continue;
+            while (i >= seg_off[s + 1]) ++s;
+            if (!C.skip) {
+                gfloat* pp = reinterpret_cast<gfloat*>(static_cast<unsigned long long>(A.segs[3 * s])) + (i - seg_off[s]);
+                float p = *pp, g = A.grad[i], m = A.m[i], v = A.v[i];
+                adam_one<false>(p, g, m, v, C);
+                *pp = p;
+                A.m[i] = m;
+                A.v[i] = v;
+            }
+            if (A.zero_grad) A.grad[i] = 0.f;
+        }
+    }
+}
+
+__device__ __forceinline__ float form_update_one(const AdamArgs& A, const AdamConsts& C, bool upd, bool zg, gfloat* pp, long long fi,
+                                                 bool fused) {
+    float p = *pp;
+    if (upd) {
+        float g = A.grad[fi], m = A.m[fi], v = A.v[fi];
+        if (fused) adam_one<true>(p, g, m, v, C);
+        else adam_one<false>(p, g, m, v, C);
+        *pp = p;
+        A.m[fi] = m;
+        A.v[fi] = v;
+    }
+    if (zg) A.grad[fi] = 0.f;
+    return p;
+}
+
+template <bool FORMS>
+__global__ __launch_bounds__(256) __attribute__((amdgpu_waves_per_eu(FORMS ? 4 : 1))) void adam_flat_kernel(const AdamArgs A) {
     __shared__ long long seg_off[kMaxSegs + 1];
     __shared__ AdamConsts consts;
-    for (int i = threadIdx.x; i < A.nseg; i += 256) seg_off[i] = A.segs[3 * i + 1];
-    if (threadIdx.x == 0) {
+    const int tid = threadIdx.x;
+    const bool tile_job = FORMS && (int)blockIdx.x < A.tile_jobs;
+    if (!tile_job)
+        for (int i = tid; i < A.nseg; i += 256) seg_off[i] = A.segs[3 * i + 1];
+    if (tid == 0) {
         seg_off[A.nseg] = A.n;
-        AdamConsts c;
-        c.skip = (A.found_inf != nullptr && A.found_inf[0] != 0.f) || (A.finite != nullptr && !isfinite(A.finite[0])) ||
-                 (A.norm != nullptr && !isfinite(A.norm[0]));
-        if (blockIdx.x == 0 && A.applied != nullptr) A.applied[0] = c.skip ? 0.f : 1.f;
-        double lr = A.lr, beta1 = A.beta1, beta2 = A.beta2, eps = A.eps, wd = A.weight_decay;
-        float max_norm = A.max_norm;
-        if (A.hyper != nullptr) {
-            lr = A.hyper[0]; beta1 = A.hyper[1]; beta2 = A.hyper[2]; eps = A.hyper[3]; wd = A.hyper[4];
-            max_norm = (float)A.hyper[5];
-        }
-        const double t = (double)A.step[0] + 1.0;
-        const double bc1 = 1.0 - pow(beta1, t), bc2 = 1.0 - pow(beta2, t);
-        c.step_size = (float)(lr / bc1);
-        c.bc2_sqrt = (float)sqrt(bc2);
-        c.beta2f = (float)beta2;
-        c.omb1 = (float)(1.0 - beta1);
-        c.omb2 = (float)(1.0 - beta2);
-        c.eps = (float)eps;
-        c.weight_decay = (float)wd;
-        c.clip = 1.f;
-        if (A.norm != nullptr) c.clip = fminf(max_norm / (A.norm[0] + 1e-6f), 1.f);
+        AdamConsts c{};
+        if (!FORMS || A.update) {
+            c.skip = (A.found_inf != nullptr && A.found_inf[0] != 0.f) || (A.finite != nullptr && !isfinite(A.finite[0])) ||
+                     (A.norm != nullptr && !isfinite(A.norm[0]));
+            if (blockIdx.x == 0 && A.applied != nullptr) A.applied[0] = c.skip ? 0.f : 1.f;
+            double lr = A.lr, beta1 = A.beta1, beta2 = A.beta2, eps = A.eps, wd = A.weight_decay;
+            float max_norm = A.max_norm;
+            if (A.hyper != nullptr) {
+                lr = A.hyper[0]; beta1 = A.hyper[1]; beta2 = A.hyper[2]; eps = A.hyper[3]; wd = A.hyper[4];
+                max_norm = (float)A.hyper[5];
+            }
+            const double t = (double)A.step[0] + 1.0;
+            const double bc1 = 1.0 - pow(beta1, t), bc2 = 1.0 - pow(beta2, t);
+            c.step_size = (float)(lr / bc1);
+            c.bc2_sqrt = (float)sqrt(bc2);
+            c.beta2f = (float)beta2;
+            c.omb1 = (float)(1.0 - beta1);
+            c.omb2 = (float)(1.0 - beta2);
+            c.eps = (float)eps;
+            c.weight_decay = (float)wd;
+            c.clip = 1.f;
+            if (A.norm != nullptr) c.clip = fminf(max_norm / (A.norm[0] + 1e-6f), 1.f);
+        }
         consts = c;
     }
     __syncthreads();
     const AdamConsts C = consts;
-    const long long n4 = (A.n + 3) >> 2;
-    for (long long q = (long long)blockIdx.x * 256 + threadIdx.x; q < n4; q += (long long)gridDim.x * 256) {
-        const long long i0 = q << 2;
-        int lo = 0, hi = A.nseg - 1;
-        while (lo < hi) {
-            const int mid = (lo + hi + 1) >> 1;
-            if (seg_off[mid] <= i0) lo = mid; else hi = mid - 1;
-        }
-        const bool full = i0 + 4 <= A.n;
-        if (full && i0 + 4 <= seg_off[lo + 1]) {
-            gfloat* pp = reinterpret_cast<gfloat*>(static_cast<unsigned long long>(A.segs[3 * lo])) + (i0 - seg_off[lo]);
-            float4 g = *reinterpret_cast<float4*>(A.grad + i0);
-            if (!C.skip) {
-                float4 m = *reinterpret_cast<float4*>(A.m + i0), v = *reinterpret_cast<float4*>(A.v + i0);
-                const bool al = (reinterpret_cast<unsigned long long>(pp) & 15) == 0;
-                float4 p;
-                if (al) {
-                    const f32x4v q = *reinterpret_cast<gf32x4*>(pp);
-                    p = float4{q[0], q[1], q[2], q[3]};
-                } else {
-                    p = float4{pp[0], pp[1], pp[2], pp[3]};
-                }
-                adam_one(p.x, g.x, m.x, v.x, C);
-                adam_one(p.y, g.y, m.y, v.y, C);
-                adam_one(p.z, g.z, m.z, v.z, C);
-                adam_one(p.w, g.w, m.w, v.w, C);
-                if (al) *reinterpret_cast<gf32x4*>(pp) = f32x4v{p.x, p.y, p.z, p.w};
-                else { pp[0] = p.x; pp[1] = p.y; pp[2] = p.z; pp[3] = p.w; }
-                *reinterpret_cast<float4*>(A.m + i0) = m;
-                *reinterpret_cast<float4*>(A.v + i0) = v;
-            }
-            if (A.zero_grad) *reinterpret_cast<float4*>(A.grad + i0) = float4{0.f, 0.f, 0.f, 0.f};
-        } else {
-            int s = lo;
-            for (int e = 0; e < 4 && i0 + e < A.n; ++e) {
-                const long long i = i0 + e;
-                while (i >= seg_off[s + 1]) ++s;
-                if (!C.skip) {
-                    gfloat* pp = reinterpret_cast<gfloat*>(static_cast<unsigned long long>(A.segs[3 * s])) + (i - seg_off[s]);
-                    float p = *pp, g = A.grad[i], m = A.m[i], v = A.v[i];
-                    adam_one(p, g, m, v, C);
-                    *pp = p;
-                    A.m[i] = m;
-                    A.v[i] = v;
-                }
-                if (A.zero_grad) A.grad[i] = 0.f;
-            }
+    if constexpr (!FORMS) {
+        const long long n4 = (A.n + 3) >> 2;
+        for (long long q = (long long)blockIdx.x * 256 + tid; q < n4; q += (long long)gridDim.x * 256) adam_quad(A, C, seg_off, q << 2, 0, A.n);
+    } else {
+        if (!tile_job) {
+            __shared__ long long ranges[3 * kMaxRestRanges];
+            for (int i = tid; i < 3 * A.nranges; i += 256) ranges[i] = A.ranges[i];
+            __syncthreads();
+            const long long nblk = (long long)gridDim.x - A.tile_jobs;
+            for (long long rq = ((long long)blockIdx.x - A.tile_jobs) * 256 + tid; rq < A.rest_quads; rq += nblk * 256) {
+                long long vlo, vhi;
+                const long long i0 = form_rest_quad(ranges, A.nranges, rq, vlo, vhi);
+                adam_quad(A, C, seg_off, i0, vlo, vhi);
+            }
+            return;
+        }
+        __shared__ __attribute__((aligned(16))) float tile[4 * 32 * 33];
+        __shared__ unsigned red[4];
+        const int blk = blockIdx.x;
+        int l = 0;
+        while (l + 1 < A.nlayers && blk >= A.layers[(l + 1) * FW_WORDS + FW_JOB_START]) ++l;
+        const long long* L = A.layers + (size_t)l * FW_WORDS;
+        const FormGeom g = form_geom((int)L[FW_H], (int)L[FW_I], (int)L[FW_KP], L[FW_PLANES_DX] ? (int)L[FW_KB_COUNT] : 0);
+        const bool upd = A.update && !C.skip, zg = A.update && A.zero_grad;
+        guint* amax = reinterpret_cast<guint*>(static_cast<unsigned long long>(L[FW_AMAX]));
+        int job = blk - (int)L[FW_JOB_START];
+        if (job < g.jobs_hh) {
+            gfloat* P = reinterpret_cast<gfloat*>(static_cast<unsigned long long>(L[FW_P_WHH]));
+            gfloat* w_pad = reinterpret_cast<gfloat*>(static_cast<unsigned long long>(L[FW_W_PAD]));
+            gfloat* w_t = reinterpret_cast<gfloat*>(static_cast<unsigned long long>(L[FW_W_T]));
+            const long long off = L[FW_OFF_WHH];
+            const int tx = tid & 31, ty = tid >> 5;
+            float m = 0.f;
+#pragma unroll
+            for (int half = 0; half < 2; ++half) {
+                float pv[8], gv[8], mv[8], vv[8];
+#pragma unroll
+                for (int e = 0; e < 8; ++e) {
+                    int row, col;
+                    pv[e] = gv[e] = mv[e] = vv[e] = 0.f;
+                    if (form_hh_elem(g, job, tid, half * 2 + (e >> 2), e & 3, row, col)) {
+                        const long long idx = (long long)row * g.H + col;
+                        pv[e] = P[idx];
+                        if (upd) {
+                            gv[e] = A.grad[off + idx];
+                            mv[e] = A.m[off + idx];
+                            vv[e] = A.v[off + idx];
+                        }
+                    }
+                }
+#pragma unroll
+                for (int e = 0; e < 8; ++e) {
+                    int row, col;
+                    const int s = half * 2 + (e >> 2), q = e & 3;
+                    const bool own = form_hh_elem(g, job, tid, s, q, row, col);
+                    if (own) {
+                        const long long idx = (long long)row * g.H + col;
+                        if (upd) {
+                            if (adam_fused_at(off + idx, off, off + (long long)g.G * g.H)) adam_one<true>(pv[e], gv[e], mv[e], vv[e], C);
+                            else adam_one<false>(pv[e], gv[e], mv[e], vv[e], C);
+                            P[idx] = pv[e];
+                            A.m[off + idx] = mv[e];
+                            A.v[off + idx] = vv[e];
+                        }
+                        if (zg) A.grad[off + idx] = 0.f;
+                    }
+                    if (row < g.G && col < g.KP) w_pad[(size_t)row * g.KP + col] = pv[e];
+                    tile[(s * 32 + ty + q * 8) * 33 + tx] = pv[e];
+                    m = fmaxf(m, fabsf(pv[e]));
+                }
+            }
+            __syncthreads();
+            const int tg = job / g.strips_h, ts = job - tg * g.strips_h;
+#pragma unroll
+            for (int s = 0; s < 4; ++s) {
+#pragma unroll
+                for (int q = 0; q < 4; ++q) {
+                    const int h = ts * 128 + s * 32 + ty + q * 8, gr = tg * 32 + tx;
+                    if (h < g.H && gr < g.G) w_t[(size_t)h * g.G + gr] = tile[(s * 32 + tx) * 33 + ty + q * 8];
+                }
+            }
+            publish_max_global(amax + 1, m, red);
+            return;
+        }
+        job -= g.jobs_hh;
+        if (job < g.jobs_ih) {
+            constexpr int P = 68;
+            gfloat* W = reinterpret_cast<gfloat*>(static_cast<unsigned long long>(L[FW_P_WIH]));
+            gfloat* cat = reinterpret_cast<gfloat*>(static_cast<unsigned long long>(L[FW_W_IH_CAT]));
+            gu32x4* planes = reinterpret_cast<gu32x4*>(static_cast<unsigned long long>(L[FW_PLANES_DX]));
+            const long long off = L[FW_OFF_WIH];
+            const int Ipad = (int)L[FW_IPAD];
+            const int lx = tid & 15, ly = tid >> 4;
+            int kb = 0, cblock = 0;
+            float m = 0.f;
+#pragma unroll
+            for (int p = 0; p < 2; ++p) {
+                int row, col;
+                form_ih_quad(g, job, tid, p, kb, cblock, row, col);
+                float z[4] = {0.f, 0.f, 0.f, 0.f};
+                if (row < g.G && col < g.I) {
+                    const long long idx = (long long)row * g.I + col, fi = off + idx;
+                    gfloat* pp = W + idx;
+                    if (col + 4 <= g.I && (fi & 3) == 0 && (reinterpret_cast<unsigned long long>(pp) & 15) == 0) {
+                        const f32x4v q = *reinterpret_cast<gf32x4*>(pp);
+                        float4 pv = float4{q[0], q[1], q[2], q[3]};
+                        if (upd) {
+                            float4 gv = *reinterpret_cast<float4*>(A.grad + fi), mv = *reinterpret_cast<float4*>(A.m + fi),
+                                   vv = *reinterpret_cast<float4*>(A.v + fi);
+                            adam_one<true>(pv.x, gv.x, mv.x, vv.x, C);
+                            adam_one<true>(pv.y, gv.y, mv.y, vv.y, C);
+                            adam_one<true>(pv.z, gv.z, mv.z, vv.z, C);
+                            adam_one<true>(pv.w, gv.w, mv.w, vv.w, C);
+                            *reinterpret_cast<gf32x4*>(pp) = f32x4v{pv.x, pv.y, pv.z, pv.w};
+                            *reinterpret_cast<float4*>(A.m + fi) = mv;
+                            *reinterpret_cast<float4*>(A.v + fi) = vv;
+                        }
+                        if (zg) *reinterpret_cast<float4*>(A.grad + fi) = float4{0.f, 0.f, 0.f, 0.f};
+                        z[0] = pv.x; z[1] = pv.y; z[2] = pv.z; z[3] = pv.w;
+                    } else {
+#pragma unroll
+                        for (int e = 0; e < 4; ++e)
+                            if (col + e < g.I)
+                                z[e] = form_update_one(A, C, upd, zg, pp + e, fi + e, adam_fused_at(fi + e, off, off + (long long)g.G * g.I));
+                    }
+                }
+                if (cat != nullptr && row < g.G && col < Ipad)
+                    *reinterpret_cast<gf32x4*>(cat + (size_t)row * Ipad + col) = f32x4v{z[0], z[1], z[2], z[3]};
+                m = fmaxf(fmaxf(m, fmaxf(fabsf(z[0]), fabsf(z[1]))), fmaxf(fabsf(z[2]), fabsf(z[3])));
+                if (planes != nullptr) *reinterpret_cast<f32x4v*>(&tile[(ly + p * 16) * P + lx * 4]) = f32x4v{z[0], z[1], z[2], z[3]};
+            }
+            if (planes != nullptr) {
+                __syncthreads();
+                const int rl = tid >> 6, g4 = (tid >> 4) & 3, r = tid & 15;
+                const long long rt = (long long)cblock * 4 + rl;
+                if (rt * 16 < ((g.I + 15) / 16) * 16) {
+                    float v[8];
+#pragma unroll
+                    for (int e = 0; e < 8; ++e) v[e] = tile[(g4 * 8 + e) * P + rl * 16 + r];
+                    u32x4 hi, lo;
+                    split_chunk_values<true>(v, hi, lo);
+                    gu32x4* o = planes + ((rt * L[FW_KB_TOTAL] + L[FW_KB_OFFSET] + kb) * 2) * FR + g4 * 16 + r;
+                    o[0] = hi;
+                    o[FR] = lo;
+                }
+            }
+            publish_max_global(amax, m, red);
+            return;
+        }
+        job -= g.jobs_ih;
+        const int idx = job * 256 + tid;
+        if (idx < g.G) {
+            const float bi = form_update_one(A, C, upd, zg, reinterpret_cast<gfloat*>(static_cast<unsigned long long>(L[FW_P_BIH])) + idx,
+                                             L[FW_OFF_BIH] + idx, adam_fused_at(L[FW_OFF_BIH] + idx, L[FW_OFF_BIH], L[FW_OFF_BIH] + g.G));
+            const float bh = form_update_one(A, C, upd, zg, reinterpret_cast<gfloat*>(static_cast<unsigned long long>(L[FW_P_BHH])) + idx,
+                                             L[FW_OFF_BHH] + idx, adam_fused_at(L[FW_OFF_BHH] + idx, L[FW_OFF_BHH], L[FW_OFF_BHH] + g.G));
+            reinterpret_cast<gfloat*>(static_cast<unsigned long long>(L[FW_BIAS]))[idx] = bi + bh;
         }
     }
 }
@@ -200,6 +477,62 @@
 }
 
 namespace ptmi {
+
+static int plan_forms(long long* layers, int nlayers, const long long* segs, int nseg, long long n, std::vector<long long>& ranges,
+                      int counts[4], long long& rest_quads) {
+    PTMI_RETURN_IF(nlayers < 0 || (nlayers > 0 && layers == nullptr) || segs == nullptr || nseg < 1 || n < 1, PTMI_E_INVALID);
+    PTMI_RETURN_IF(nlayers > kMaxFormLayers, PTMI_E_UNSUPPORTED);
+    std::vector<std::pair<long long, long long>> owned;
+    counts[0] = counts[1] = counts[2] = counts[3] = 0;
+    long long jobs = 0;
+    for (int l = 0; l < nlayers; ++l) {
+        long long* L = layers + (size_t)l * FW_WORDS;
+        const long long H = L[FW_H], I = L[FW_I], KP = L[FW_KP];
+        PTMI_RETURN_IF(H < 1 || I < 1 || KP < H || L[FW_IPAD] < I || (L[FW_IPAD] & 3) || 4 * H * std::max(I, KP) >= (1ll << 31), PTMI_E_INVALID);
+        PTMI_RETURN_IF(!L[FW_W_PAD] || !L[FW_W_T] || !L[FW_BIAS] || !L[FW_AMAX], PTMI_E_INVALID);
+        PTMI_RETURN_IF((L[FW_W_IH_CAT] & 15) || (L[FW_PLANES_DX] & 15), PTMI_E_INVALID);
+        if (L[FW_PLANES_DX])
+            PTMI_RETURN_IF(L[FW_KB_COUNT] < (4 * H + 31) / 32 || L[FW_KB_OFFSET] < 0 || L[FW_KB_OFFSET] + L[FW_KB_COUNT] > L[FW_KB_TOTAL],
+                           PTMI_E_INVALID);
+        const long long count[4] = {4 * H * I, 4 * H * H, 4 * H, 4 * H};
+        for (int k = 0; k < 4; ++k) {
+            bool found = false;
+            for (int s = 0; s < nseg && !found; ++s)
+                found = segs[3 * s] == L[FW_P_WIH + k] && segs[3 * s + 1] == L[FW_OFF_WIH + k] && segs[3 * s + 2] == count[k];
+            PTMI_RETURN_IF(!found || L[FW_OFF_WIH + k] < 0 || L[FW_OFF_WIH + k] + count[k] > n, PTMI_E_INVALID);
+            owned.emplace_back(L[FW_OFF_WIH + k], L[FW_OFF_WIH + k] + count[k]);
+        }
+        const FormGeom g = form_geom((int)H, (int)I, (int)KP, L[FW_PLANES_DX] ? (int)L[FW_KB_COUNT] : 0);
+        L[FW_JOB_START] = jobs;
+        jobs += (long long)g.jobs_hh + g.jobs_ih + g.jobs_bias;
+        L[FW_JOB_END] = jobs;
+        counts[0] += g.jobs_hh;
+        counts[1] += g.jobs_ih;
+        counts[2] += g.jobs_bias;
+        PTMI_RETURN_IF(jobs >= (1ll << 30), PTMI_E_UNSUPPORTED);
+    }
+    std::sort(owned.begin(), owned.end());
+    ranges.clear();
+    rest_quads = 0;
+    long long at = 0;
+    auto rest = [&](long long lo, long long hi) {
+        if (lo >= hi) return;
+        ranges.push_back(lo);
+        ranges.push_back(hi);
+        ranges.push_back(rest_quads);
+        rest_quads += ((hi + 3) >> 2) - (lo >> 2);
+    };
+    for (const auto& o : owned) {
+        PTMI_RETURN_IF(o.first < at, PTMI_E_INVALID);
+        rest(at, o.first);
+        at = o.second;
+    }
+    rest(at, n);
+    PTMI_RETURN_IF((int)(ranges.size() / 3) > kMaxRestRanges, PTMI_E_UNSUPPORTED);
+    const long long blocks = (rest_quads + 255) / 256;
+    counts[3] = (int)(blocks < 8192 ? blocks : 8192);
+    return PTMI_OK;
+}
 
 }
 
@@ -234,8 +567,102 @@
     const long long n4 = (n + 3) >> 2;
     const long long blocks = (n4 + 255) / 256;
     const int grid = (int)(blocks < 8192 ? blocks : 8192);
-    hipLaunchKernelGGL(adam_flat_kernel, dim3(grid), dim3(256), 0, static_cast<hipStream_t>(stream), A);
+    hipLaunchKernelGGL(adam_flat_kernel<false>, dim3(grid), dim3(256), 0, static_cast<hipStream_t>(stream), A);
     return launch_status();
 }
 
-}
+int ptmi_adam_forms_plan(int64_t* layers, int32_t nlayers, const int64_t* segments, int32_t nseg, int64_t n, int64_t* ranges,
+                         int32_t* nranges, int32_t* counts, int64_t* rest_quads) {
+    PTMI_RETURN_IF(ranges == nullptr || nranges == nullptr || counts == nullptr || rest_quads == nullptr, PTMI_E_INVALID);
+    std::vector<long long> r;
+    int c[4];
+    long long rq = 0;
+    const int rc = plan_forms(reinterpret_cast<long long*>(layers), nlayers, reinterpret_cast<const long long*>(segments), nseg, n, r, c, rq);
+    if (rc != PTMI_OK) return rc;
+    for (size_t i = 0; i < r.size(); ++i) ranges[i] = r[i];
+    *nranges = (int32_t)(r.size() / 3);
+    for (int i = 0; i < 4; ++i) counts[i] = c[i];
+    *rest_quads = rq;
+    return PTMI_OK;
+}
+
+int ptmi_adam_forms_owners(const int64_t* layers_, int32_t nlayers, const int64_t* segments, int32_t nseg, int64_t n, int32_t* owner,
+                           int64_t* conflicts) {
+    PTMI_RETURN_IF(owner == nullptr || conflicts == nullptr, PTMI_E_INVALID);
+    std::vector<long long> layers(layers_, layers_ + (size_t)std::max(nlayers, 0) * FW_WORDS), ranges;
+    int counts[4];
+    long long rest_quads = 0, bad = 0;
+    const int rc = plan_forms(layers.data(), nlayers, reinterpret_cast<const long long*>(segments), nseg, n, ranges, counts, rest_quads);
+    if (rc != PTMI_OK) return rc;
+    for (long long i = 0; i < n; ++i) owner[i] = -1;
+    auto claim = [&](long long i, int job) {
+        if (i < 0 || i >= n || owner[i] != -1) ++bad;
+        else owner[i] = job;
+    };
+    for (int l = 0; l < nlayers; ++l) {
+        const long long* L = layers.data() + (size_t)l * FW_WORDS;
+        const FormGeom g = form_geom((int)L[FW_H], (int)L[FW_I], (int)L[FW_KP], L[FW_PLANES_DX] ? (int)L[FW_KB_COUNT] : 0);
+        int blk = (int)L[FW_JOB_START];
+        for (int job = 0; job < g.jobs_hh; ++job, ++blk)
+            for (int tid = 0; tid < 256; ++tid)
+                for (int e = 0; e < 16; ++e) {
+                    int row, col;
+                    if (form_hh_elem(g, job, tid, e >> 2, e & 3, row, col)) claim(L[FW_OFF_WHH] + (long long)row * g.H + col, blk);
+                }
+        for (int job = 0; job < g.jobs_ih; ++job, ++blk)
+            for (int tid = 0; tid < 256; ++tid)
+                for (int p = 0; p < 2; ++p) {
+                    int kb, cblock, row, col;
+                    form_ih_quad(g, job, tid, p, kb, cblock, row, col);
+                    for (int e = 0; e < 4; ++e)
+                        if (row < g.G && col + e < g.I) claim(L[FW_OFF_WIH] + (long long)row * g.I + col + e, blk);
+                }
+        for (int job = 0; job < g.jobs_bias; ++job, ++blk)
+            for (int tid = 0; tid < 256; ++tid)
+                if (job * 256 + tid < g.G) {
+                    claim(L[FW_OFF_BIH] + job * 256 + tid, blk);
+                    claim(L[FW_OFF_BHH] + job * 256 + tid, blk);
+                }
+        if (blk != (int)L[FW_JOB_END]) ++bad;
+    }
+    const int tile_jobs = counts[0] + counts[1] + counts[2], nranges = (int)(ranges.size() / 3);
+    for (long long rq = 0; rq < rest_quads; ++rq) {
+        long long vlo, vhi;
+        const long long i0 = form_rest_quad(ranges.data(), nranges, rq, vlo, vhi);
+        for (int e = 0; e < 4; ++e)
+            if (i0 + e >= vlo && i0 + e < vhi) claim(i0 + e, tile_jobs + (int)((rq / 256) % counts[3]));
+    }
+    *conflicts = bad;
+    return PTMI_OK;
+}
+
+int ptmi_adam_flat_forms(float* flat_grad, float* exp_avg, float* exp_avg_sq, const int64_t* segments, int32_t nseg, int64_t n,
+                         const float* norm, float max_norm, const float* found_inf, const float* finite, float* applied, const float* step,
+                         double lr, double beta1, double beta2, double eps, double weight_decay, const double* hyper, int32_t zero_grad,
+                         const int64_t* layers, int32_t nlayers, const int64_t* ranges, int32_t nranges, int32_t tile_jobs,
+                         int32_t rest_blocks, int64_t rest_quads, uint32_t* amax_words, int32_t n_amax_words, int32_t update,
+                         ptmi_stream_t stream) {
+    PTMI_RETURN_IF(segments == nullptr || nseg < 1 || n < 1 || nlayers < 0 || nranges < 0 || tile_jobs < 0 || rest_blocks < 0, PTMI_E_INVALID);
+    PTMI_RETURN_IF(nseg > kMaxSegs || nlayers > kMaxFormLayers || nranges > kMaxRestRanges, PTMI_E_UNSUPPORTED);
+    PTMI_RETURN_IF((nlayers > 0 && (layers == nullptr || amax_words == nullptr)) || (nranges > 0 && ranges == nullptr), PTMI_E_INVALID);
+    if (update) {
+        PTMI_RETURN_IF(flat_grad == nullptr || exp_avg == nullptr || exp_avg_sq == nullptr || step == nullptr, PTMI_E_INVALID);
+        PTMI_RETURN_IF(((reinterpret_cast<uintptr_t>(flat_grad) | reinterpret_cast<uintptr_t>(exp_avg) |
+                         reinterpret_cast<uintptr_t>(exp_avg_sq)) & 15) != 0, PTMI_E_INVALID);
+        PTMI_RETURN_IF((reinterpret_cast<uintptr_t>(hyper) & 7) != 0, PTMI_E_INVALID);
+        PTMI_RETURN_IF((rest_quads > 0) != (rest_blocks > 0), PTMI_E_INVALID);
+    }
+    AdamArgs A{flat_grad, exp_avg, exp_avg_sq, reinterpret_cast<const long long*>(segments), nseg, (long long)n, norm, max_norm,
+               found_inf, finite, applied, step, lr, beta1, beta2, eps, weight_decay, hyper, zero_grad,
+               reinterpret_cast<const long long*>(layers), reinterpret_cast<const long long*>(ranges), nlayers, nranges, tile_jobs,
+               (long long)rest_quads, update ? 1 : 0};
+    hipStream_t st = static_cast<hipStream_t>(stream);
+    hipError_t e = zero_words_async(amax_words, (size_t)n_amax_words, st);
+    if (e != hipSuccess) return (int)e;
+    const long long grid = (long long)tile_jobs + (update ? rest_blocks : 0);
+    if (grid == 0) return PTMI_OK;
+    hipLaunchKernelGGL(adam_flat_kernel<true>, dim3((unsigned)grid), dim3(256), 0, st, A);
+    return launch_status();
+}
+
+}
diff --git a/padertorch_amd/csrc/planes_chunk.h b/padertorch_amd/csrc/planes_chunk.h
--- /dev/null
+++ b/padertorch_amd/csrc/planes_chunk.h
@@ -0,0 +1,43 @@
+#pragma once
+#include <hip/hip_runtime.h>
+
+namespace ptmi {
+
+typedef _Float16 h8 __attribute__((ext_vector_type(8)));
+typedef __bf16 b8 __attribute__((ext_vector_type(8)));
+typedef unsigned u32x4 __attribute__((ext_vector_type(4)));
+
+constexpr int FR = 64;
+
+template <bool BF16>
+__device__ __forceinline__ void split_chunk_values(const float (&v)[8], u32x4& hi_out, u32x4& lo_out) {
+    if (BF16) {
+        b8 hi, lo;
+#pragma unroll
+        for (int e = 0; e < 8; ++e) {
+            hi[e] = (__bf16)v[e];
+            lo[e] = (__bf16)(v[e] - (float)hi[e]);
+        }
+        hi_out = __builtin_bit_cast(u32x4, hi);
+        lo_out = __builtin_bit_cast(u32x4, lo);
+    } else {
+        h8 hi, lo;
+#pragma unroll
+        for (int e = 0; e < 8; ++e) {
+            hi[e] = (_Float16)v[e];
+            lo[e] = (_Float16)(v[e] - (float)hi[e]);
+        }
+        hi_out = __builtin_bit_cast(u32x4, hi);
+        lo_out = __builtin_bit_cast(u32x4, lo);
+    }
+}
+
+template <bool BF16>
+__device__ __forceinline__ void split_chunk(const float (&v)[8], uint4* hi_out, uint4* lo_out) {
+    u32x4 hi, lo;
+    split_chunk_values<BF16>(v, hi, lo);
+    *hi_out = __builtin_bit_cast(uint4, hi);
+    *lo_out = __builtin_bit_cast(uint4, lo);
+}
+
+}
diff --git a/padertorch_amd/ops/gemm.py b/padertorch_amd/ops/gemm.py
--- a/padertorch_amd/ops/gemm.py
+++ b/padertorch_amd/ops/gemm.py
@@ -51,6 +51,12 @@
 
 
 def invalidate():
+    _drop()
+    from . import lstm_forms as _forms
+    _forms.forget_written()
+
+
+def _drop():
     _WEIGHT_AMAX.clear()
     _WEIGHT_PLANES.clear()
     _UPDATED.clear()
@@ -61,7 +67,7 @@
 
 def reset_step():
     known = dict(_KNOWN)
-    invalidate()
+    _drop()
     _KNOWN.update(known)
     _WAITED.clear()
 
diff --git a/padertorch_amd/ops/library.py b/padertorch_amd/ops/library.py
--- a/padertorch_amd/ops/library.py
+++ b/padertorch_amd/ops/library.py
@@ -657,6 +657,27 @@
                           exp_avg_sq.data_ptr(), segments.data_ptr(), segments.shape[0], flat_grad.numel(), _lib.ptr(norm),
                           max_norm, _lib.ptr(found_inf), _lib.ptr(finite), applied.data_ptr(), step.data_ptr(), lr, beta1, beta2,
                           eps, weight_decay, _lib.ptr(hyper), int(zero_grad), _lib.stream(flat_grad.device)), 'ptmi_adam_flat')
+    return applied
+
+
+@_register('adam_flat_forms_(Tensor(a!) flat_grad, Tensor(b!) exp_avg, Tensor(c!) exp_avg_sq, Tensor segments, Tensor(d!)[] params, '
+           'Tensor? norm, float max_norm, Tensor? found_inf, Tensor? finite, Tensor step, float lr, float beta1, float beta2, '
+           'float eps, float weight_decay, bool zero_grad, Tensor? hyper, Tensor layers, Tensor ranges, int[] plan, '
+           'Tensor(e!) amax_words, Tensor(f!)[] forms, bool update) -> Tensor')
+def adam_flat_forms_(flat_grad, exp_avg, exp_avg_sq, segments, params, norm, max_norm, found_inf, finite, step, lr, beta1, beta2, eps,
+                     weight_decay, zero_grad, hyper, layers, ranges, plan, amax_words, forms, update):
+    if hyper is not None:
+        assert hyper.dtype == torch.float64 and hyper.numel() >= 6 and hyper.device == flat_grad.device and hyper.is_contiguous(), hyper
+    assert layers.dtype == torch.int64 and ranges.dtype == torch.int64 and layers.is_contiguous() and ranges.is_contiguous()
+    assert layers.device == flat_grad.device and ranges.device == flat_grad.device and amax_words.dtype == torch.int32
+    applied = torch.empty((), dtype=torch.float32, device=flat_grad.device)
+    tile_jobs, rest_blocks, rest_quads = plan
+    _lib.check(_lib.timed('adam_flat', _lib.load().ptmi_adam_flat_forms, flat_grad.data_ptr(), exp_avg.data_ptr(),
+                          exp_avg_sq.data_ptr(), segments.data_ptr(), segments.shape[0], flat_grad.numel(), _lib.ptr(norm),
+                          max_norm, _lib.ptr(found_inf), _lib.ptr(finite), applied.data_ptr(), step.data_ptr(), lr, beta1, beta2,
+                          eps, weight_decay, _lib.ptr(hyper), int(zero_grad), layers.data_ptr(), layers.shape[0], ranges.data_ptr(),
+                          ranges.shape[0], tile_jobs, rest_blocks, rest_quads, amax_words.data_ptr(), amax_words.numel(), int(update),
+                          _lib.stream(flat_grad.device)), 'ptmi_adam_flat_forms')
     return applied
 
 
diff --git a/padertorch_amd/ops/lstm_forms.py b/padertorch_amd/ops/lstm_forms.py
--- a/padertorch_amd/ops/lstm_forms.py
+++ b/padertorch_amd/ops/lstm_forms.py
@@ -1,15 +1,27 @@
+import ctypes
+import weakref
+
 import torch
 
 from .. import _lib
 from . import gemm as _gemm
 
+FROM_OPTIMIZER = True
+
 _STACKED = {}
+_REGISTERED = {}
+_GENERATION = [0]
 _PREP_STREAMS = {}
 _EARLY_FORK = {}
 
 
 def clear():
     _STACKED.clear()
+
+
+def forget_written():
+    for reg in _REGISTERED.values():
+        reg.valid = None
 
 
 def reset_step():
@@ -51,13 +63,13 @@
 
 class _LazyPlanes:
 
-    def __init__(self, w, amax):
-        self.w, self.amax, self.value = w, amax, None
+    def __init__(self, w, amax, make=None):
+        self.w, self.amax, self.value, self.make = w, amax, None, make
 
     def get(self):
         if self.value is None:
             with torch.no_grad():
-                self.value = _gemm.pack_n(self.w, self.amax)
+                self.value = _gemm.pack_n(self.w, self.amax) if self.make is None else self.make()
         return self.value
 
 
@@ -117,6 +129,187 @@
         w_t=w_hh.transpose(1, 2).contiguous())
 
 
+def _sig(params):
+    return tuple((p._version, p.data_ptr()) for ps in params for p in ps)
+
+
+def _wants_dx(ndir, H, I, dx_from_handoff):
+    if not (_gemm.planes_enabled() and dx_from_handoff and I == ndir * H):
+        return 0
+    return int(_lib.load().ptmi_lstm_handoff_cols(H, 1))
+
+
+class _Registered:
+
+    def __init__(self, params, KP, cols_dx):
+        self.refs = tuple(tuple(weakref.ref(p) for p in ps) for ps in params)
+        self.ndir, (self.G, self.I), self.H, self.KP, self.cols_dx = len(params), params[0][0].shape, params[0][1].shape[1], KP, cols_dx
+        self.Ipad = (self.I + 3) // 4 * 4
+        self.device = params[0][0].device
+        self.w_ih_cat = self.bias = self.w_pad = self.w_t = self.amax = self.planes_dx = None
+        self.valid = self.owner = None
+
+    def params(self):
+        ps = tuple(tuple(r() for r in rs) for rs in self.refs)
+        return None if any(p is None for q in ps for p in q) else ps
+
+    def holds(self, params):
+        mine = self.params()
+        return mine is not None and len(mine) == len(params) and all(a is b for x, y in zip(mine, params) for a, b in zip(x, y))
+
+    def allocate(self, amax):
+        f32 = dict(dtype=torch.float32, device=self.device)
+        self.w_ih_cat, self.bias = torch.empty((self.ndir * self.G, self.Ipad), **f32), torch.empty(self.ndir * self.G, **f32)
+        self.w_pad, self.w_t = torch.empty((self.ndir, self.G, self.KP), **f32), torch.empty((self.ndir, self.H, self.G), **f32)
+        self.amax = amax
+        self.planes_dx = None
+        if self.cols_dx:
+            self.planes_dx = torch.empty((self.I + 15) // 16 * (self.ndir * self.cols_dx // 32) * 1024, dtype=torch.bfloat16, device=self.device)
+        self.valid = None
+
+    def table_rows(self, offsets):
+        rows = []
+        for d, ps in enumerate(self.params()):
+            rows.append([p.data_ptr() for p in ps] + [offsets[id(p)] for p in ps] + [self.H, self.I, self.KP, self.Ipad,
+                        self.w_pad[d].data_ptr(), self.w_t[d].data_ptr(), self.bias[d * self.G:].data_ptr(), self.amax.data_ptr(),
+                        self.w_ih_cat[d * self.G:].data_ptr(), 0 if self.planes_dx is None else self.planes_dx.data_ptr(),
+                        self.ndir * self.cols_dx // 32, d * self.cols_dx // 32, self.cols_dx // 32, 0, 0, 0])
+        return rows
+
+    def buffers(self):
+        return [t for t in (self.w_ih_cat, self.bias, self.w_pad, self.w_t, self.planes_dx) if t is not None]
+
+
+def _register(params, KP, dx_from_handoff):
+    from . import capture as _capture
+    if not FROM_OPTIMIZER or _capture.ACTIVE:
+        return
+    key = tuple(id(p) for ps in params for p in ps)
+    p0 = params[0][0]
+    cols_dx = _wants_dx(len(params), params[0][1].shape[1], p0.shape[1], dx_from_handoff)
+    reg = _REGISTERED.get(key)
+    if reg is not None and reg.holds(params) and (reg.KP, reg.cols_dx) == (KP, cols_dx):
+        return
+    for k in [k for k, r in _REGISTERED.items() if r.params() is None]:
+        del _REGISTERED[k]
+    _REGISTERED[key] = _Registered(params, KP, cols_dx)
+    _GENERATION[0] += 1
+
+
+def _pack_rows(w_list, amax, blocks=None):
+    G, I = w_list[0].shape
+    assert G % 16 == 0, G
+    if blocks is None:
+        kb_total = (I + 31) // 32
+        col_blocks = [(0, I, 0, kb_total)]
+    else:
+        ndir, H, cols = blocks
+        assert cols % 32 == 0 and I == ndir * H, (cols, I, ndir, H)
+        kb_total = ndir * cols // 32
+        col_blocks = [(d * H, (d + 1) * H, d * cols // 32, cols // 32) for d in range(ndir)]
+    out = torch.empty(len(w_list) * G // 16 * kb_total * 1024, dtype=torch.float16, device=w_list[0].device)
+    for r, w in enumerate(w_list):
+        rows_out = out[r * (G // 16) * kb_total * 1024:]
+        for c0, c1, kbo, kbn in col_blocks:
+            torch.ops.ptmi.pack_planes_into_(rows_out, w[:, c0:c1], amax, False, kb_total, kbo, kbn)
+    return out
+
+
+def _forms_registered(reg, params, stream):
+    main = torch.cuda.current_stream(reg.device)
+    ndir, H, I = reg.ndir, reg.H, reg.I
+    amax = reg.amax
+    w_list = [ps[0].detach() for ps in params]
+    with torch.cuda.stream(stream if stream is not None else main):
+        planes = planes_h = None
+        cols_ = int(_lib.load().ptmi_lstm_handoff_cols(H, 0)) if _gemm.planes_enabled() else 0
+        if cols_ and I == ndir * H:
+            planes_h = ((_pack_rows(w_list, amax[0:1], (ndir, H, cols_)), amax[0:1]), cols_)
+            if cols_ == H:
+                planes = planes_h[0]
+        if _gemm.planes_enabled() and planes is None:
+            if planes_h is None:
+                planes = (_pack_rows(w_list, amax[0:1]), amax[0:1])
+            else:
+                planes = _LazyPlanes(None, amax[0:1], lambda: (_pack_rows(w_list, amax[0:1]), amax[0:1]))
+        planes_dx = (reg.planes_dx, reg.cols_dx) if (planes is not None and reg.planes_dx is not None) else None
+    w_ih_k = reg.w_ih_cat
+    forms = LayerForms(w_ih_k[:, :I], reg.bias, reg.w_pad[:, :, :H], reg.w_pad, reg.w_t, w_ih_k if reg.Ipad != I else None,
+                       planes, planes_h, planes_dx)
+    if stream is not None:
+        forms.ready = torch.cuda.Event()
+        forms.ready.record(stream)
+    _gemm.seed_weights_absmax([ps[0] for ps in params], amax[0:1])
+    _gemm.seed_weights_absmax([ps[1] for ps in params], amax[1:2])
+    return forms
+
+
+def _registered_valid(params, KP, dx_from_handoff):
+    if not FROM_OPTIMIZER:
+        return None
+    reg = _REGISTERED.get(tuple(id(p) for ps in params for p in ps))
+    if reg is None or reg.valid is None or reg.valid != _sig(params) or not reg.holds(params):
+        return None
+    p0 = params[0][0]
+    if (reg.KP, reg.cols_dx) != (KP, _wants_dx(len(params), params[0][1].shape[1], p0.shape[1], dx_from_handoff)):
+        return None
+    return reg
+
+
+class OptimizerForms:
+
+    def __init__(self, layers, flat_params, offsets, segs, n):
+        ids = {id(p): off for p, off in zip(flat_params, offsets)}
+        self.layers = layers
+        self.amax_words = torch.zeros(max(2 * len(self.layers), 1), dtype=torch.int32, device=segs.device)
+        rows = []
+        for i, reg in enumerate(self.layers):
+            reg.allocate(self.amax_words[2 * i:2 * i + 2])
+            reg.owner = self
+            rows += reg.table_rows(ids)
+        words = int(_lib.PTMI_ADAM_FORMS_LAYER_WORDS)
+        table = torch.tensor(rows, dtype=torch.int64).reshape(len(rows), words)
+        segs_host = segs.cpu().contiguous()
+        ranges = torch.zeros((64, 3), dtype=torch.int64)
+        nranges, counts, rest_quads = ctypes.c_int32(0), (ctypes.c_int32 * 4)(), ctypes.c_int64(0)
+        _lib.check(_lib.load().ptmi_adam_forms_plan(table.data_ptr(), table.shape[0], segs_host.data_ptr(), segs_host.shape[0], int(n),
+                                                    ranges.data_ptr(), ctypes.byref(nranges), counts, ctypes.byref(rest_quads)),
+                   'ptmi_adam_forms_plan')
+        self.counts = tuple(int(c) for c in counts)
+        self.plan = [sum(self.counts[:3]), self.counts[3], int(rest_quads.value)]
+        self.table_host, self.ranges_host = table, ranges[:nranges.value].contiguous()
+        self.table, self.ranges = table.to(segs.device), self.ranges_host.to(segs.device)
+        self.buffers = [t for reg in self.layers for t in reg.buffers()]
+
+    def mark_written(self):
+        for reg in self.layers:
+            ps = reg.params()
+            if reg.owner is self:
+                reg.valid = None if ps is None else _sig(ps)
+
+    def stale(self):
+        return any(reg.owner is not self or ((ps := reg.params()) is not None and reg.valid != _sig(ps)) for reg in self.layers)
+
+
+def optimizer_forms(cached, bound, flat_params):
+    from . import capture as _capture
+    if not FROM_OPTIMIZER:
+        return None
+    if cached is not None and cached[0] is bound and cached[1] == _GENERATION[0]:
+        return cached
+    if _capture.ACTIVE:
+        return None
+    m, _, _, segs, _, offs = bound
+    ids = {id(p) for p in flat_params}
+    layers = [reg for reg in _REGISTERED.values()
+              if (ps := reg.params()) is not None and reg.device == segs.device
+              and all(id(p) in ids and p.is_contiguous() and p.dtype == torch.float32 for q in ps for p in q)][:32]
+    if cached is not None and cached[0] is bound and (cached[2].layers if cached[2] is not None else []) == layers \
+            and all(reg.owner is cached[2] for reg in layers):
+        return (bound, _GENERATION[0], cached[2])
+    return (bound, _GENERATION[0], OptimizerForms(layers, flat_params, offs, segs, m.numel()) if layers else None)
+
+
 def stacked_weights(params, KP, dx_from_handoff, stream=None):
     key = tuple(id(p) for ps in params for p in ps)
     sig = tuple((p._version, p.data_ptr()) for ps in params for p in ps)
@@ -128,7 +321,12 @@
         _STACKED.clear()
     with torch.no_grad():
         if params[0][0].is_cuda and all(p.dtype == torch.float32 and p.is_contiguous() for ps in params for p in ps):
-            forms = _forms_kernel(params, KP, dx_from_handoff, stream)
+            reg = _registered_valid(params, KP, dx_from_handoff)
+            if reg is not None:
+                forms = _forms_registered(reg, params, stream)
+            else:
+                forms = _forms_kernel(params, KP, dx_from_handoff, stream)
+                _register(params, KP, dx_from_handoff)
         else:
             forms = _forms_torch(params, KP)
     _STACKED[key] = (sig, forms, _gemm._refs(flat_ps))
diff --git a/padertorch_amd/train/graphed.py b/padertorch_amd/train/graphed.py
--- a/padertorch_amd/train/graphed.py
+++ b/padertorch_amd/train/graphed.py
@@ -258,6 +258,7 @@
                 opt.hyper_from_device = False
         self._graph = graph
         self._device_hyper = device_hyper
+        self._forms = getattr(opt, 'forms_last_step', None) if device_hyper else None
         self._baked = None if device_hyper else self._baked_hyper()
         self._pattern = self._weight_pattern()
         self.captures += 1
@@ -276,6 +277,8 @@
             tr.optimizer.refresh_device_hyper(self.device)
         if tr.loss_weights is not None:
             self._stage.refresh_loss_weights(tr.loss_weights)
+        if self._forms is not None and self._forms.stale():
+            tr.optimizer.refresh_forms(self._forms)
 
     def load(self, examples):
         assert len(examples) == len(self.examples), (len(examples), len(self.examples))
@@ -314,6 +317,8 @@
         tr._opt_step += 1
         self._steps += 1
         torch.autograd.graph.increment_version(tr._flat.params)
+        if self._forms is not None:
+            self._forms.mark_written()
         torch.cuda.current_stream(self.device).synchronize()
         if self.split and self.times is not None:
             self.times.append(tuple(ev[i].elapsed_time(ev[i + 1]) for i in range(3)))
diff --git a/padertorch_amd/train/optimizer.py b/padertorch_amd/train/optimizer.py
--- a/padertorch_amd/train/optimizer.py
+++ b/padertorch_amd/train/optimizer.py
@@ -115,10 +115,13 @@
         self.skip_if_not_finite = None
         self._hyper = None
         self.hyper_from_device = False
+        self._forms = None
+        self.forms_last_step = None
 
     def set_parameters(self, parameters):
         self.parameters = tuple(parameters)
         self._bound = None
+        self._forms = self.forms_last_step = None
         try:
             self.optimizer = self.optimizer_cls(self.parameters, fused=True, **self.optimizer_kwargs)
         except (RuntimeError, TypeError, ValueError):
@@ -190,6 +193,14 @@
         return self._norm
 
     @torch.no_grad()
+    def refresh_forms(self, forms):
+        m, v, steps, segs, _, _ = self._bound
+        fg = self.flat_grads
+        torch.ops.ptmi.adam_flat_forms_(fg.flat, m, v, segs, list(fg.params), None, 0.0, None, None, steps, 0.0, 0.0, 0.0, 0.0, 0.0, False,
+                                        None, forms.table, forms.ranges, forms.plan, forms.amax_words, forms.buffers, False)
+        forms.mark_written()
+
+    @torch.no_grad()
     def _native_step(self, zero_grad):
         m, v, steps, segs, _, _ = self._bind()
         fg, opt = self.flat_grads, self.optimizer
@@ -201,12 +212,20 @@
         if finite is not None:
             finite = finite.detach().reshape(1).float()
         hyper = self._hyper[1] if self.hyper_from_device else None
-        applied = torch.ops.ptmi.adam_flat_(
-            fg.flat, m, v, segs, list(fg.params), self._norm, float(self.gradient_clipping),
-            None if found is None else found.reshape(1).float(), finite, steps, float(g['lr']), float(g['betas'][0]),
-            float(g['betas'][1]), float(g['eps']), float(g['weight_decay']), bool(zero_grad), hyper)
+        from ..ops import gemm as _gemm, lstm_forms as _forms
+        self._forms = _forms.optimizer_forms(self._forms, self._bound, fg.params)
+        forms = self._forms[2] if self._forms is not None else None
+        args = (fg.flat, m, v, segs, list(fg.params), self._norm, float(self.gradient_clipping),
+                None if found is None else found.reshape(1).float(), finite, steps, float(g['lr']), float(g['betas'][0]),
+                float(g['betas'][1]), float(g['eps']), float(g['weight_decay']), bool(zero_grad), hyper)
+        if forms is not None:
+            applied = torch.ops.ptmi.adam_flat_forms_(*args, forms.table, forms.ranges, forms.plan, forms.amax_words, forms.buffers, True)
+        else:
+            applied = torch.ops.ptmi.adam_flat_(*args)
         torch.autograd.graph.increment_version(fg.params)
-        from ..ops import gemm as _gemm
+        if forms is not None:
+            forms.mark_written()
+        self.forms_last_step = forms
         _gemm.note_update(fg.params)
         steps.add_(applied)
         self._norm = None
```
